# sotelo/parrot

Hardware: AMD Instinct MI355X
Metric: acoustic feature frames/sec (train fwd+bwd+allreduce+clip/Adam) (higher is better)
Workload: dtype f32; 1 GPU; BASELINE configs[1]: 2-layer attention-GRU decoder, h=1024, batch=64 per GPU, T_enc=200, T_dec=800, fp32; cell=gru, layers=2, hidden=1024, batch_per_gpu=64, global_batch=64, T_enc=200, T_dec=800, parallelism=dp1, params=13919212

## Files before the change

### include/parrot_hip.h

```cpp
#ifndef PARROT_HIP_H
#define PARROT_HIP_H

#include <stddef.h>
#include <stdint.h>

#ifdef __cplusplus
extern "C" {
#endif

#define PARROT_ERR_BADARG 10001
#define PARROT_ERR_UNSUPPORTED 10002

#define PARROT_NORM_EPS 1e-5f
#define PARROT_MAX_LAYERS 3

const char* parrot_hip_version(void);

int parrot_profile_begin(void);
long long parrot_profile_end(double* total_us, double* flops, double* bytes);
long long parrot_profile_end2(double* total_us, double* flops, double* bytes, double* plain4);

#define PARROT_PRECISION_F32 0
#define PARROT_PRECISION_BF16 1
#define PARROT_PRECISION_BF16X3 2
int parrot_set_gemm_precision(int mode);
int parrot_get_gemm_precision(void);
int parrot_gemm(const float* A, int lda, int transA, const float* B, int ldb, int transB, float* C, int ldc,
                int M, int N, int K, const float* bias, float alpha, int accumulate, int act, int nbatch,
                long long strideA, long long strideB, long long strideC, int split_k, void* stream);

int parrot_gemm_gated(const float* A, int lda, int transA, const float* B, int ldb, int transB, float* C, int ldc,
                      int M, int N, int K, const float* gate, int ldg, void* stream);

#define PARROT_GEMM_ROUTE_STEP 0
#define PARROT_GEMM_ROUTE_F32 1
#define PARROT_GEMM_ROUTE_BF16 2
#define PARROT_GEMM_ROUTE_BF16X3 3
int parrot_gemm_route(const float* A, int lda, int transA, const float* B, int ldb, int transB, int M, int N, int K,
                      float alpha, int act, int nbatch, long long strideA, long long strideB, int split_k, int has_gate,
                      int* kernel, int* slices);

int parrot_to_bf16(const float* x, void* y, long long n, void* stream);
int parrot_gemm_bf16in(const void* A, int lda, const void* B, int ldb, float* C, int ldc, int M, int N, int K,
                       int accumulate, int split_k, void* stream);
int parrot_gemm_bf16in_ex(const void* A, int lda, int transA, const void* B, int ldb, int transB, float* C, int ldc, int M,
                          int N, int K, const float* bias, int accumulate, int split_k, void* stream);

int parrot_colsum(const float* x, long long M, int N, int ld, float* out, int accumulate, void* stream);

int parrot_gru_step_fwd(const float* h, const float* inputs, const float* gate_inputs, const float* mask,
                        const float* Wg, const float* Wc, float* h_out, float* z, float* r, float* rh,
                        float* c, int B, int H, void* stream);

int parrot_gru_step_bwd(const float* dh_out, const float* h, const float* mask, const float* Wg,
                        const float* Wc, const float* z, const float* r, const float* c, float* dh,
                        float* d_inputs, float* d_gate_inputs, int B, int H, void* stream);

typedef struct ParrotGruSeqDesc {
    int T, B, H, nchain, use_graph, reserved;
    int reverse[4];
    const float* Wg[4];
    const float* Wc[4];
    const float* inputs[4];
    const float* gate_inputs[4];
    const float* mask;
    float* h[4];
    float* z[4]; float* r[4]; float* rh[4]; float* c[4];
    float* dh[4];
    float* dG[4];
    float* dC[4];
} ParrotGruSeqDesc;

int parrot_gru_seq_create(const ParrotGruSeqDesc* desc, void** plan);
int parrot_gru_seq_fwd(void* plan, void* stream);
int parrot_gru_seq_bwd(void* plan, void* stream);
int parrot_gru_seq_destroy(void* plan);

typedef struct ParrotLstmSeqDesc {
    int T, B, H, use_graph;
    const float* W;
    const float* pre_in;
    float* s; float* c;
    float* gates;
    float* dS;
    float* dc;
    float* dP;
} ParrotLstmSeqDesc;

int parrot_lstm_seq_create(const ParrotLstmSeqDesc* desc, void** plan);
int parrot_lstm_seq_fwd(void* plan, void* stream);
int parrot_lstm_seq_bwd(void* plan, void* stream);
int parrot_lstm_seq_destroy(void* plan);

int parrot_gmm_attention_fwd(const float* h1, const float* WattT, const float* batt, const float* kappa_prev,
                             const float* ctx, float* a, float* b, float* kappa, float* phi, float* w, int B,
                             int H, int A, int U, int E, int att_type, float eps, float alignment,
                             float sharpening, float timing, void* stream);

int parrot_gmm_attention_bwd(const float* dw, const float* ctx, const float* a, const float* b,
                             const float* kappa, const float* kappa_prev, const float* WattT, float* dkappa,
                             float* dp, float* dh1, int B, int H, int A, int U, int E, int att_type, float eps,
                             void* stream);

typedef struct ParrotDecoderDesc {
    int T, B, H, E, A, U, L, att_type, use_graph;
    int reserved;
    float eps, alignment, sharpening, timing;
    const float* Wg[PARROT_MAX_LAYERS];
    const float* Wc[PARROT_MAX_LAYERS];
    const float* bg[PARROT_MAX_LAYERS];
    const float* bc[PARROT_MAX_LAYERS];
    const float* WattT;
    const float* batt;
    const float* ctx;
    float* seq_c[PARROT_MAX_LAYERS];
    float* seq_g[PARROT_MAX_LAYERS];
    float* h[PARROT_MAX_LAYERS];
    float* w;
    float* kappa;
    float* z[PARROT_MAX_LAYERS]; float* r[PARROT_MAX_LAYERS];
    float* rh[PARROT_MAX_LAYERS]; float* c[PARROT_MAX_LAYERS];
    float* a; float* b;
    float* phi;
    float* dh[PARROT_MAX_LAYERS];
    float* dw;
    float* dw0;
    float* dhup[PARROT_MAX_LAYERS];
    float* dkappa;
    float* dG[PARROT_MAX_LAYERS];
    float* dC[PARROT_MAX_LAYERS];
    float* dp;
    int cell;
    int seq_init;
    float* cst[PARROT_MAX_LAYERS];
    float* gate4[PARROT_MAX_LAYERS];
    float* dcell[PARROT_MAX_LAYERS];
    int layer_norm, bf16;
    const float* ln_bg[PARROT_MAX_LAYERS * PARROT_MAX_LAYERS];
    const float* ln_bc[PARROT_MAX_LAYERS * PARROT_MAX_LAYERS];
    float* ln_yg[PARROT_MAX_LAYERS * PARROT_MAX_LAYERS];
    float* ln_yc[PARROT_MAX_LAYERS * PARROT_MAX_LAYERS];
    float* ln_sg[PARROT_MAX_LAYERS * PARROT_MAX_LAYERS];
    float* ln_sc[PARROT_MAX_LAYERS * PARROT_MAX_LAYERS];
    const float* Wg_f[PARROT_MAX_LAYERS];
    const float* Wc_f[PARROT_MAX_LAYERS];
    const float* Wg_r[PARROT_MAX_LAYERS];
    const float* Wc_r[PARROT_MAX_LAYERS];
    int* att_sup;
    float* persist_ws;
    long long persist_ws_floats;
    float* dh_b[PARROT_MAX_LAYERS];
    float* dhup_b[PARROT_MAX_LAYERS];
    float* dw_b;
    float* dw0_b;
    float* dhup_c[PARROT_MAX_LAYERS];
    float* dw_c;
    float* dw0_c;
    void* dG16[PARROT_MAX_LAYERS];
} ParrotDecoderDesc;

long long parrot_decoder_persist_floats(const ParrotDecoderDesc* desc);
int parrot_decoder_is_persistent(void* plan);
int parrot_decoder_schedule(void* plan);
int parrot_decoder_backward_tick(void* plan);
long long parrot_decoder_trace(void* plan, int which, long long* out, long long cap);
long long parrot_decoder_trace_jobs(void* plan, int which, long long* out, long long cap);
int parrot_decoder_status(void* plan);

int parrot_decoder_create(const ParrotDecoderDesc* desc, void** plan);
int parrot_decoder_writes_bf16_grads(void* plan);
int parrot_decoder_seq_fwd(void* plan, void* stream);
int parrot_decoder_seq_bwd(void* plan, void* stream);
int parrot_decoder_destroy(void* plan);

#define PARROT_READOUT_MAX_SEG 4
typedef struct ParrotReadoutComposedDesc {
    long long M;
    long long ws_floats;
    int nseg, R, O, zero_rows;
    int slice_rows, nbias;
    int K[PARROT_READOUT_MAX_SEG];
    int ldx[PARROT_READOUT_MAX_SEG];
    int lddx[PARROT_READOUT_MAX_SEG];
    int ldwr, ldwo, ldp, lddp;
    int ldgwr, ldgwo;
    const float* x[PARROT_READOUT_MAX_SEG];
    const float* Wr; const float* Wo;
    const float* rb[PARROT_READOUT_MAX_SEG];
    const float* bo;
    float* pred;
    const float* dp;
    float* dx[PARROT_READOUT_MAX_SEG];
    float* gWr; float* gWo;
    float* grb[PARROT_READOUT_MAX_SEG];
    float* gbo;
} ParrotReadoutComposedDesc;

long long parrot_readout_composed_ws_floats(const ParrotReadoutComposedDesc* desc);
int parrot_readout_composed_fwd(const ParrotReadoutComposedDesc* desc, float* ws, void* stream);
int parrot_readout_composed_bwd(const ParrotReadoutComposedDesc* desc, float* ws, void* stream);

typedef struct ParrotSampleDesc {
    int S, B, H, E, A, U, L, O, R, ldx, att_type, use_graph;
    float eps, alignment, sharpening, timing;
    const float* Wg[PARROT_MAX_LAYERS];
    const float* Wc[PARROT_MAX_LAYERS];
    const float* bg[PARROT_MAX_LAYERS];
    const float* bc[PARROT_MAX_LAYERS];
    const float* Wfg[PARROT_MAX_LAYERS];
    const float* Wfc[PARROT_MAX_LAYERS];
    const float* seq_c[PARROT_MAX_LAYERS];
    const float* seq_g[PARROT_MAX_LAYERS];
    const float* WattT; const float* batt;
    const float* Wr; const float* br;
    const float* radd;
    const float* Wo; const float* bo;
    const float* oadd;
    const float* ctx;
    float* x;
    float* h[PARROT_MAX_LAYERS];
    float* w;
    float* kappa;
    float* a;
    float* bwork;
    float* phi;
    float* zwork; float* rwork; float* rhwork; float* readout;
    int gmm_K, reserved2;
    float sampling_bias, reserved3;
    const float* Wmu; const float* bmu; const float* Wsig; const float* bsig; const float* Wco; const float* bco;
    const float* add_mu; const float* add_sig; const float* add_co;
    const float* unif; const float* noise;
    float* gmm_mu; float* gmm_sig; float* gmm_co;
    float* pi_out;
    int cell, reserved5;
    float* cwork[PARROT_MAX_LAYERS];
    float* gwork;
    int layer_norm, reserved7;
    const float* bfg[PARROT_MAX_LAYERS];
    const float* bfc[PARROT_MAX_LAYERS];
    const float* ln_bg[PARROT_MAX_LAYERS * PARROT_MAX_LAYERS];
    const float* ln_bc[PARROT_MAX_LAYERS * PARROT_MAX_LAYERS];
    const float* br_l[PARROT_MAX_LAYERS];
    float* ln_scratch;
    long long ln_scratch_floats;
    const float* Wg_t[PARROT_MAX_LAYERS];
    const float* Wc_t[PARROT_MAX_LAYERS];
    const float* Wr_t; const float* Wo_t; const float* bo_pad; const float* oadd_pad;
    float* persist_ws;
    long long persist_ws_floats;
    const float* Wro_t;
    const float* ro_const;
    const float* Wgx_t[PARROT_MAX_LAYERS];
    const float* Wcx_t[PARROT_MAX_LAYERS];
    const float* Watt_t;
    int bf16, reserved8;
    const void* Wg_t16[PARROT_MAX_LAYERS];
    const int* eou_pos;
    const int* eou_ncmp;
    int* eou_first;
    int eou_extra, reserved9;
} ParrotSampleDesc;

long long parrot_sample_persist_floats(const ParrotSampleDesc* desc);
int parrot_sample_is_persistent(void* plan);
int parrot_sample_is_bf16(void* plan);
int parrot_sample_plan_pieces_dry(const ParrotSampleDesc* desc, int nwg, int* info16);
int parrot_sample_status(void* plan);
int parrot_sample_stops_early(void* plan);
int parrot_sample_steps_run(void* plan, int* steps);

int parrot_sample_create(const ParrotSampleDesc* desc, void** plan);
int parrot_sample_run(void* plan, void* stream);
int parrot_sample_destroy(void* plan);

int parrot_plan_last_error(void* plan);

int parrot_sumsq(const float* x, size_t n, float* out, void* stream);

int parrot_tile_weights(const float* W, int rows, int cols, int ld, float* out, int mode, int lstm_H, void* stream);
int parrot_tile_weights_bf16(const float* W, int rows, int cols, int ld, void* out, int mode, int lstm_H, void* stream);

int parrot_simple_norm_fwd(const float* x, int ldx, float* y, int ldy, float* sigma, long long R, int N, float eps,
                           float* add_dst, int ld_add, void* stream);
int parrot_simple_norm_bwd(const float* dy, int lddy, const float* y, int ldy, const float* sigma, float* dx,
                           int lddx, long long R, int N, float eps, int accumulate, void* stream);
int parrot_adam_clip_step(float* param, const float* grad, float* m, float* v, size_t n,
                          const float* gnorm_sq, float grad_scale, float clip_threshold, float lr,
                          float beta1, float beta2, float eps, int step, void* stream);

int parrot_batch_quantize(const float* x, int rows, int n, int ld, double* ws, void* out, int ldo, int mode,
                          int q_levels, void* stream);
int parrot_mu2linear(const int32_t* q, size_t n, float* out, void* stream);

int parrot_gather_sum_fwd(const float* tbl, const int* idx, const float* add, int ldadd, float* y, int ldy, long long N,
                          int J, int Q, int D, void* stream);
long long parrot_gather_sum_bwd_ws_floats(long long N, int J, int Q, int D);
int parrot_gather_sum_bwd(const float* dy, int lddy, const int* perm, const int* offs, float* dtbl, float* ws,
                          long long ws_floats, long long N, int J, int Q, int D, int accumulate, void* stream);
int parrot_softmax_ce_fwd(const float* logits, int ld, const int* target, long long rows, int Q, float* lse, float* ce,
                          void* stream);
int parrot_softmax_ce_bwd(const float* logits, int ld, const int* target, const float* lse, const float* rowscale,
                          long long rows, int Q, float* dlogits, int ldd, void* stream);
int parrot_relu_gate(const float* dy, const float* gate, float* out, long long n, void* stream);

int parrot_gmm_cost_fwd(const float* y, int ldy, const float* mu, int ldmu, const float* sig_hat, int ldsig,
                        const float* co_hat, int ldco, long long M, int O, int K, float eps, float* nll, float* pi_out,
                        int ldpi, float* logr, void* stream);
int parrot_gmm_cost_bwd(const float* y, int ldy, const float* mu, int ldmu, const float* sig_hat, int ldsig,
                        const float* co_hat, int ldco, const float* logr, const float* rowscale, long long M, int O, int K,
                        float eps, float* dmu, int lddmu, float* dsig_hat, int lddsig, float* dco_hat, int lddco,
                        void* stream);

long long samplernn_weightnorm_ws_floats(int N);
int samplernn_weightnorm_fold(const float* W, int ld, const float* g, float* W_eff, int ldo, float* norm, float* ws, int K, int N,
                              void* stream);
int samplernn_weightnorm_fold_bwd(const float* W, int ld, const float* g, const float* norm, const float* dW_eff, int ldd,
                                  float* dW, int lddw, float* dg, float* ws, int K, int N, int accumulate_w, int accumulate_g,
                                  void* stream);

typedef struct SampleRnnGenDesc {
    int B, D, T, Q, FS, BFS, feat_dim, use_graph;
    float temperature; int reserved;
    unsigned long long seed;
    const float* big_Win_frames; const float* big_Win_feats; const float* big_bin;
    const float* big_U; const float* big_bU; const float* big_Wg; const float* big_Wc;
    const float* big_Wout; const float* big_bout;
    const float* frm_Win; const float* frm_bin;
    const float* frm_U; const float* frm_bU; const float* frm_Wg; const float* frm_Wc;
    const float* frm_Wout; const float* frm_bout;
    const float* emb_tbl;
    const float* W2; const float* b2; const float* W3; const float* b3; const float* W4; const float* b4;
    const float* features;
    int* samples;
    float* big_h; float* frm_h;
    float* xf_big; float* xf_frm; float* feat_cur; float* gru_in; float* P; float* z; float* r; float* rh;
    float* big_out; float* frame_out; float* o1; float* o2; float* o3; float* logits;
    int* tbase;
    int n_rnn, lstm;
    const float* big_L[5][4];
    const float* frm_L[5][4];
    float* big_hs[5]; float* big_cs[5];
    float* frm_hs[5]; float* frm_cs[5];
    float* gate_ws; float* layer_tmp;
    float* persist_ws;
    long long persist_ws_floats;
} SampleRnnGenDesc;

long long samplernn_persist_floats(const SampleRnnGenDesc* desc);
int samplernn_generate_create(const SampleRnnGenDesc* desc, void** plan);
int samplernn_generate_run(void* plan, void* stream);
int samplernn_generate_is_persistent(void* plan);
int samplernn_generate_status(void* plan);
int samplernn_generate_destroy(void* plan);

#ifdef __cplusplus
}
#endif
#endif
```

### parrot_amd/_lib.py

```python
from __future__ import annotations

import ctypes as C
import os

from .utils import env_str

_HERE = os.path.dirname(os.path.abspath(__file__))
LIB_PATH = os.path.join(_HERE, "libparrot_hip.so")

MAX_LAYERS = 3

c_float_p = C.c_void_p


class HipLibraryMissing(RuntimeError):
    pass


class HipCallError(RuntimeError):
    pass


class GruSeqDesc(C.Structure):
    _fields_ = [
        ("T", C.c_int), ("B", C.c_int), ("H", C.c_int), ("nchain", C.c_int),
        ("use_graph", C.c_int), ("reserved", C.c_int),
        ("reverse", C.c_int * 4),
        ("Wg", C.c_void_p * 4), ("Wc", C.c_void_p * 4),
        ("inputs", C.c_void_p * 4), ("gate_inputs", C.c_void_p * 4),
        ("mask", C.c_void_p),
        ("h", C.c_void_p * 4),
        ("z", C.c_void_p * 4), ("r", C.c_void_p * 4), ("rh", C.c_void_p * 4), ("c", C.c_void_p * 4),
        ("dh", C.c_void_p * 4), ("dG", C.c_void_p * 4), ("dC", C.c_void_p * 4),
    ]


class LstmSeqDesc(C.Structure):
    _fields_ = [(n, C.c_int) for n in ("T", "B", "H", "use_graph")] + \
               [(n, C.c_void_p) for n in ("W", "pre_in", "s", "c", "gates", "dS", "dc", "dP")]


class DecoderDesc(C.Structure):
    _fields_ = [
        ("T", C.c_int), ("B", C.c_int), ("H", C.c_int), ("E", C.c_int), ("A", C.c_int),
        ("U", C.c_int), ("L", C.c_int), ("att_type", C.c_int), ("use_graph", C.c_int),
        ("reserved", C.c_int),
        ("eps", C.c_float), ("alignment", C.c_float), ("sharpening", C.c_float), ("timing", C.c_float),
        ("Wg", C.c_void_p * MAX_LAYERS), ("Wc", C.c_void_p * MAX_LAYERS),
        ("bg", C.c_void_p * MAX_LAYERS), ("bc", C.c_void_p * MAX_LAYERS),
        ("WattT", C.c_void_p), ("batt", C.c_void_p), ("ctx", C.c_void_p),
        ("seq_c", C.c_void_p * MAX_LAYERS), ("seq_g", C.c_void_p * MAX_LAYERS),
        ("h", C.c_void_p * MAX_LAYERS), ("w", C.c_void_p), ("kappa", C.c_void_p),
        ("z", C.c_void_p * MAX_LAYERS), ("r", C.c_void_p * MAX_LAYERS),
        ("rh", C.c_void_p * MAX_LAYERS), ("c", C.c_void_p * MAX_LAYERS),
        ("a", C.c_void_p), ("b", C.c_void_p), ("phi", C.c_void_p),
        ("dh", C.c_void_p * MAX_LAYERS), ("dw", C.c_void_p), ("dw0", C.c_void_p), ("dhup", C.c_void_p * MAX_LAYERS),
        ("dkappa", C.c_void_p),
        ("dG", C.c_void_p * MAX_LAYERS), ("dC", C.c_void_p * MAX_LAYERS), ("dp", C.c_void_p),
        ("cell", C.c_int), ("seq_init", C.c_int),
        ("cst", C.c_void_p * MAX_LAYERS), ("gate4", C.c_void_p * MAX_LAYERS), ("dcell", C.c_void_p * MAX_LAYERS),
        ("layer_norm", C.c_int), ("bf16", C.c_int),
        ("ln_bg", C.c_void_p * (MAX_LAYERS * MAX_LAYERS)), ("ln_bc", C.c_void_p * (MAX_LAYERS * MAX_LAYERS)),
        ("ln_yg", C.c_void_p * (MAX_LAYERS * MAX_LAYERS)), ("ln_yc", C.c_void_p * (MAX_LAYERS * MAX_LAYERS)),
        ("ln_sg", C.c_void_p * (MAX_LAYERS * MAX_LAYERS)), ("ln_sc", C.c_void_p * (MAX_LAYERS * MAX_LAYERS)),
        ("Wg_f", C.c_void_p * MAX_LAYERS), ("Wc_f", C.c_void_p * MAX_LAYERS),
        ("Wg_r", C.c_void_p * MAX_LAYERS), ("Wc_r", C.c_void_p * MAX_LAYERS),
        ("att_sup", C.c_void_p),
        ("persist_ws", C.c_void_p), ("persist_ws_floats", C.c_longlong),
        ("dh_b", C.c_void_p * MAX_LAYERS), ("dhup_b", C.c_void_p * MAX_LAYERS), ("dw_b", C.c_void_p), ("dw0_b", C.c_void_p),
        ("dhup_c", C.c_void_p * MAX_LAYERS), ("dw_c", C.c_void_p), ("dw0_c", C.c_void_p),
        ("dG16", C.c_void_p * MAX_LAYERS),
    ]


READOUT_MAX_SEG = 4


class ReadoutComposedDesc(C.Structure):
    _fields_ = [
        ("M", C.c_longlong), ("ws_floats", C.c_longlong),
        ("nseg", C.c_int), ("R", C.c_int), ("O", C.c_int), ("zero_rows", C.c_int),
        ("slice_rows", C.c_int), ("nbias", C.c_int),
        ("K", C.c_int * READOUT_MAX_SEG), ("ldx", C.c_int * READOUT_MAX_SEG), ("lddx", C.c_int * READOUT_MAX_SEG),
        ("ldwr", C.c_int), ("ldwo", C.c_int), ("ldp", C.c_int), ("lddp", C.c_int),
        ("ldgwr", C.c_int), ("ldgwo", C.c_int),
        ("x", C.c_void_p * READOUT_MAX_SEG),
        ("Wr", C.c_void_p), ("Wo", C.c_void_p),
        ("rb", C.c_void_p * READOUT_MAX_SEG), ("bo", C.c_void_p),
        ("pred", C.c_void_p), ("dp", C.c_void_p),
        ("dx", C.c_void_p * READOUT_MAX_SEG),
        ("gWr", C.c_void_p), ("gWo", C.c_void_p),
        ("grb", C.c_void_p * READOUT_MAX_SEG), ("gbo", C.c_void_p),
    ]


class SampleDesc(C.Structure):
    _fields_ = [
        ("S", C.c_int), ("B", C.c_int), ("H", C.c_int), ("E", C.c_int), ("A", C.c_int),
        ("U", C.c_int), ("L", C.c_int), ("O", C.c_int), ("R", C.c_int), ("ldx", C.c_int),
        ("att_type", C.c_int), ("use_graph", C.c_int),
        ("eps", C.c_float), ("alignment", C.c_float), ("sharpening", C.c_float), ("timing", C.c_float),
        ("Wg", C.c_void_p * MAX_LAYERS), ("Wc", C.c_void_p * MAX_LAYERS),
        ("bg", C.c_void_p * MAX_LAYERS), ("bc", C.c_void_p * MAX_LAYERS),
        ("Wfg", C.c_void_p * MAX_LAYERS), ("Wfc", C.c_void_p * MAX_LAYERS),
        ("seq_c", C.c_void_p * MAX_LAYERS), ("seq_g", C.c_void_p * MAX_LAYERS),
        ("WattT", C.c_void_p), ("batt", C.c_void_p),
        ("Wr", C.c_void_p), ("br", C.c_void_p), ("radd", C.c_void_p),
        ("Wo", C.c_void_p), ("bo", C.c_void_p), ("oadd", C.c_void_p),
        ("ctx", C.c_void_p),
        ("x", C.c_void_p), ("h", C.c_void_p * MAX_LAYERS), ("w", C.c_void_p), ("kappa", C.c_void_p),
        ("a", C.c_void_p), ("bwork", C.c_void_p), ("phi", C.c_void_p),
        ("zwork", C.c_void_p), ("rwork", C.c_void_p), ("rhwork", C.c_void_p), ("readout", C.c_void_p),
        ("gmm_K", C.c_int), ("reserved2", C.c_int), ("sampling_bias", C.c_float), ("reserved3", C.c_float),
        ("Wmu", C.c_void_p), ("bmu", C.c_void_p), ("Wsig", C.c_void_p), ("bsig", C.c_void_p),
        ("Wco", C.c_void_p), ("bco", C.c_void_p),
        ("add_mu", C.c_void_p), ("add_sig", C.c_void_p), ("add_co", C.c_void_p),
        ("unif", C.c_void_p), ("noise", C.c_void_p),
        ("gmm_mu", C.c_void_p), ("gmm_sig", C.c_void_p), ("gmm_co", C.c_void_p), ("pi_out", C.c_void_p),
        ("cell", C.c_int), ("reserved5", C.c_int),
        ("cwork", C.c_void_p * MAX_LAYERS), ("gwork", C.c_void_p),
        ("layer_norm", C.c_int), ("reserved7", C.c_int),
        ("bfg", C.c_void_p * MAX_LAYERS), ("bfc", C.c_void_p * MAX_LAYERS),
        ("ln_bg", C.c_void_p * (MAX_LAYERS * MAX_LAYERS)), ("ln_bc", C.c_void_p * (MAX_LAYERS * MAX_LAYERS)),
        ("br_l", C.c_void_p * MAX_LAYERS),
        ("ln_scratch", C.c_void_p), ("ln_scratch_floats", C.c_longlong),
        ("Wg_t", C.c_void_p * MAX_LAYERS), ("Wc_t", C.c_void_p * MAX_LAYERS),
        ("Wr_t", C.c_void_p), ("Wo_t", C.c_void_p), ("bo_pad", C.c_void_p), ("oadd_pad", C.c_void_p),
        ("persist_ws", C.c_void_p), ("persist_ws_floats", C.c_longlong),
        ("Wro_t", C.c_void_p), ("ro_const", C.c_void_p),
        ("Wgx_t", C.c_void_p * MAX_LAYERS), ("Wcx_t", C.c_void_p * MAX_LAYERS),
        ("Watt_t", C.c_void_p),
        ("bf16", C.c_int), ("reserved8", C.c_int),
        ("Wg_t16", C.c_void_p * MAX_LAYERS),
        ("eou_pos", C.c_void_p), ("eou_ncmp", C.c_void_p), ("eou_first", C.c_void_p),
        ("eou_extra", C.c_int), ("reserved9", C.c_int),
    ]


class SampleRnnGenDesc(C.Structure):
    _fields_ = ([(n, C.c_int) for n in ("B", "D", "T", "Q", "FS", "BFS", "feat_dim", "use_graph")] +
                [("temperature", C.c_float), ("reserved", C.c_int), ("seed", C.c_ulonglong)] +
                [(n, C.c_void_p) for n in (
                    "big_Win_frames", "big_Win_feats", "big_bin", "big_U", "big_bU", "big_Wg", "big_Wc",
                    "big_Wout", "big_bout", "frm_Win", "frm_bin", "frm_U", "frm_bU", "frm_Wg", "frm_Wc",
                    "frm_Wout", "frm_bout", "emb_tbl", "W2", "b2", "W3", "b3", "W4", "b4", "features",
                    "samples", "big_h", "frm_h", "xf_big", "xf_frm", "feat_cur", "gru_in", "P", "z", "r", "rh",
                    "big_out", "frame_out", "o1", "o2", "o3", "logits", "tbase")] +
                [("n_rnn", C.c_int), ("lstm", C.c_int),
                 ("big_L", (C.c_void_p * 4) * 5), ("frm_L", (C.c_void_p * 4) * 5),
                 ("big_hs", C.c_void_p * 5), ("big_cs", C.c_void_p * 5),
                 ("frm_hs", C.c_void_p * 5), ("frm_cs", C.c_void_p * 5),
                 ("gate_ws", C.c_void_p), ("layer_tmp", C.c_void_p),
                 ("persist_ws", C.c_void_p), ("persist_ws_floats", C.c_longlong)])


_vp, _i, _f, _ll, _sz = C.c_void_p, C.c_int, C.c_float, C.c_longlong, C.c_size_t
SIGNATURES = {
    "parrot_hip_version": (C.c_char_p, []),
    "parrot_profile_begin": (_i, []),
    "parrot_profile_end": (C.c_longlong, [C.POINTER(C.c_double)] * 3),
    "parrot_profile_end2": (C.c_longlong, [C.POINTER(C.c_double)] * 4),
    "parrot_gemm": (_i, [_vp, _i, _i, _vp, _i, _i, _vp, _i, _i, _i, _i, _vp, _f, _i, _i, _i, _ll, _ll, _ll, _i, _vp]),
    "parrot_gemm_gated": (_i, [_vp, _i, _i, _vp, _i, _i, _vp, _i, _i, _i, _i, _vp, _i, _vp]),
    "parrot_gemm_route": (_i, [_vp, _i, _i, _vp, _i, _i, _i, _i, _i, _f, _i, _i, _ll, _ll, _i, _i,
                               C.POINTER(C.c_int), C.POINTER(C.c_int)]),
    "parrot_gather_sum_fwd": (_i, [_vp, _vp, _vp, _i, _vp, _i, _ll, _i, _i, _i, _vp]),
    "parrot_gather_sum_bwd_ws_floats": (C.c_longlong, [_ll, _i, _i, _i]),
    "parrot_gather_sum_bwd": (_i, [_vp, _i, _vp, _vp, _vp, _vp, _ll, _ll, _i, _i, _i, _i, _vp]),
    "parrot_softmax_ce_fwd": (_i, [_vp, _i, _vp, _ll, _i, _vp, _vp, _vp]),
    "parrot_softmax_ce_bwd": (_i, [_vp, _i, _vp, _vp, _vp, _ll, _i, _vp, _i, _vp]),
    "parrot_relu_gate": (_i, [_vp, _vp, _vp, _ll, _vp]),
    "parrot_gmm_cost_fwd": (_i, [_vp, _i] * 4 + [_ll, _i, _i, _f, _vp, _vp, _i, _vp, _vp]),
    "parrot_gmm_cost_bwd": (_i, [_vp, _i] * 4 + [_vp, _vp, _ll, _i, _i, _f] + [_vp, _i] * 3 + [_vp]),
    "samplernn_weightnorm_ws_floats": (_ll, [_i]),
    "samplernn_weightnorm_fold": (_i, [_vp, _i, _vp, _vp, _i, _vp, _vp, _i, _i, _vp]),
    "samplernn_weightnorm_fold_bwd": (_i, [_vp, _i, _vp, _vp, _vp, _i, _vp, _i, _vp, _vp, _i, _i, _i, _i, _vp]),
    "parrot_colsum": (_i, [_vp, _ll, _i, _i, _vp, _i, _vp]),
    "parrot_gru_step_fwd": (_i, [_vp] * 11 + [_i, _i, _vp]),
    "parrot_gru_step_bwd": (_i, [_vp] * 11 + [_i, _i, _vp]),
    "parrot_gru_seq_create": (_i, [C.POINTER(GruSeqDesc), C.POINTER(C.c_void_p)]),
    "parrot_gru_seq_fwd": (_i, [_vp, _vp]),
    "parrot_gru_seq_bwd": (_i, [_vp, _vp]),
    "parrot_gru_seq_destroy": (_i, [_vp]),
    "parrot_lstm_seq_create": (_i, [C.POINTER(LstmSeqDesc), C.POINTER(C.c_void_p)]),
    "parrot_lstm_seq_fwd": (_i, [_vp, _vp]),
    "parrot_lstm_seq_bwd": (_i, [_vp, _vp]),
    "parrot_lstm_seq_destroy": (_i, [_vp]),
    "parrot_gmm_attention_fwd": (_i, [_vp] * 10 + [_i] * 6 + [_f] * 4 + [_vp]),
    "parrot_gmm_attention_bwd": (_i, [_vp] * 10 + [_i] * 6 + [_f, _vp]),
    "parrot_decoder_create": (_i, [C.POINTER(DecoderDesc), C.POINTER(C.c_void_p)]),
    "parrot_decoder_persist_floats": (C.c_longlong, [C.POINTER(DecoderDesc)]),
    "parrot_decoder_is_persistent": (_i, [_vp]),
    "parrot_decoder_schedule": (_i, [_vp]),
    "parrot_decoder_backward_tick": (_i, [_vp]),
    "parrot_decoder_writes_bf16_grads": (_i, [_vp]),
    "parrot_decoder_trace": (C.c_longlong, [_vp, _i, C.POINTER(C.c_longlong), C.c_longlong]),
    "parrot_decoder_trace_jobs": (C.c_longlong, [_vp, _i, C.POINTER(C.c_longlong), C.c_longlong]),
    "parrot_decoder_seq_fwd": (_i, [_vp, _vp]),
    "parrot_decoder_seq_bwd": (_i, [_vp, _vp]),
    "parrot_decoder_destroy": (_i, [_vp]),
    "parrot_readout_composed_ws_floats": (C.c_longlong, [C.POINTER(ReadoutComposedDesc)]),
    "parrot_readout_composed_fwd": (_i, [C.POINTER(ReadoutComposedDesc), _vp, _vp]),
    "parrot_readout_composed_bwd": (_i, [C.POINTER(ReadoutComposedDesc), _vp, _vp]),
    "parrot_sample_create": (_i, [C.POINTER(SampleDesc), C.POINTER(C.c_void_p)]),
    "parrot_sample_persist_floats": (C.c_longlong, [C.POINTER(SampleDesc)]),
    "parrot_sample_is_persistent": (_i, [_vp]),
    "parrot_sample_is_bf16": (_i, [_vp]),
    "parrot_sample_plan_pieces_dry": (_i, [C.POINTER(SampleDesc), _i, C.POINTER(C.c_int)]),
    "parrot_sample_status": (_i, [_vp]),
    "parrot_sample_stops_early": (_i, [_vp]),
    "parrot_sample_steps_run": (_i, [_vp, C.POINTER(C.c_int)]),
    "parrot_decoder_status": (_i, [_vp]),
    "parrot_sample_run": (_i, [_vp, _vp]),
    "parrot_sample_destroy": (_i, [_vp]),
    "parrot_plan_last_error": (_i, [_vp]),
    "parrot_sumsq": (_i, [_vp, _sz, _vp, _vp]),
    "parrot_tile_weights": (_i, [_vp, _i, _i, _i, _vp, _i, _i, _vp]),
    "parrot_tile_weights_bf16": (_i, [_vp, _i, _i, _i, _vp, _i, _i, _vp]),
    "parrot_set_gemm_precision": (_i, [_i]),
    "parrot_get_gemm_precision": (_i, []),
    "parrot_to_bf16": (_i, [_vp, _vp, _ll, _vp]),
    "parrot_gemm_bf16in": (_i, [_vp, _i, _vp, _i, _vp, _i, _i, _i, _i, _i, _i, _vp]),
    "parrot_gemm_bf16in_ex": (_i, [_vp, _i, _i, _vp, _i, _i, _vp, _i, _i, _i, _i, _vp, _i, _i, _vp]),
    "parrot_simple_norm_fwd": (_i, [_vp, _i, _vp, _i, _vp, _ll, _i, _f, _vp, _i, _vp]),
    "parrot_simple_norm_bwd": (_i, [_vp, _i, _vp, _i, _vp, _vp, _i, _ll, _i, _f, _i, _vp]),
    "parrot_adam_clip_step": (_i, [_vp, _vp, _vp, _vp, _sz, _vp, _f, _f, _f, _f, _f, _f, _i, _vp]),
    "parrot_batch_quantize": (_i, [_vp, _i, _i, _i, _vp, _vp, _i, _i, _i, _vp]),
    "parrot_mu2linear": (_i, [_vp, _sz, _vp, _vp]),
    "samplernn_generate_create": (_i, [C.POINTER(SampleRnnGenDesc), C.POINTER(C.c_void_p)]),
    "samplernn_generate_run": (_i, [_vp, _vp]),
    "samplernn_persist_floats": (C.c_longlong, [C.POINTER(SampleRnnGenDesc)]),
    "samplernn_generate_is_persistent": (_i, [_vp]),
    "samplernn_generate_status": (_i, [_vp]),
    "samplernn_generate_destroy": (_i, [_vp]),
}

_lib = None


def load():
    global _lib
    if _lib is not None:
        return _lib
    import torch
    path = env_str('PARROT_HIP_LIB', LIB_PATH)
    if not os.path.exists(path):
        raise HipLibraryMissing(
            f"{LIB_PATH} not found: build it with `python -m parrot_amd.build` "
            "(hipcc --offload-arch=gfx950).  There is no CPU fallback for the product path.")
    lib = C.CDLL(path)
    for name, (res, args) in SIGNATURES.items():
        fn = getattr(lib, name)
        fn.restype = res
        fn.argtypes = args
    _lib = lib
    return lib


def check(rc: int, what: str, plan=None):
    if rc != 0:
        raise HipCallError(f"{what} failed with code {rc}")


def call(name: str, *args):
    lib = load()
    rc = getattr(lib, name)(*args)
    check(rc, name)
    return rc
```

### parrot_amd/build.py

```python
from __future__ import annotations

import hashlib
import os
import subprocess
import sys
from concurrent.futures import ThreadPoolExecutor

from .utils import env_str

HERE = os.path.dirname(os.path.abspath(__file__))
CSRC = os.path.join(HERE, "csrc")
OUT = os.path.join(HERE, "libparrot_hip.so")
OBJDIR = os.path.join(CSRC, "build")
ARCH = "gfx950"

SOURCES = ["skinny.hip", "biggemm.hip", "attention.hip", "elementwise.hip", "quantize.hip",
           "plans.hip", "plans_decode.hip", "capi.hip", "samplernn.hip", "persist.hip", "sr_persist.hip", "rowgru.hip", "trainops.hip", "readout.hip",
           "gmmcost.hip"]
EXTRA_FLAGS = {"quantize.hip": ["-ffp-contract=off"]}
if env_str("PARROT_PM_DEPTH"):
    EXTRA_FLAGS["persist.hip"] = ["-DPM_DEPTH=" + env_str("PARROT_PM_DEPTH")]


def _hipcc() -> str:
    for cand in (os.environ.get("HIPCC"), "/opt/rocm/bin/hipcc", "hipcc"):
        if cand and (os.path.isabs(cand) and os.path.exists(cand) or not os.path.isabs(cand)):
            return cand
    return "hipcc"


def _digest(paths) -> str:
    h = hashlib.sha256()
    for p in sorted(paths):
        with open(p, "rb") as f:
            h.update(p.encode())
            h.update(f.read())
    return h.hexdigest()


def build(force: bool = False, verbose: bool = True, timers: bool = False) -> str:
    global OUT, OBJDIR
    if timers:
        OUT = os.path.join(HERE, "libparrot_hip_timers.so")
        OBJDIR = os.path.join(CSRC, "build_timers")
    tag, extra = env_str("PARROT_BUILD_TAG"), env_str("PARROT_BUILD_FLAGS", "").split()
    if tag:
        OUT = os.path.join(HERE, f"libparrot_hip_{tag}.so")
        OBJDIR = os.path.join(CSRC, f"build_{tag}")
    srcs = [s for s in SOURCES if os.path.exists(os.path.join(CSRC, s))]
    deps = [os.path.join(CSRC, f) for f in os.listdir(CSRC) if f.endswith((".hip", ".h"))]
    deps.append(os.path.join(HERE, "..", "include", "parrot_hip.h"))
    stamp = os.path.join(OBJDIR, "stamp.txt")
    dig = _digest(deps)
    if not force and os.path.exists(OUT) and os.path.exists(stamp) and open(stamp).read() == dig:
        return OUT
    os.makedirs(OBJDIR, exist_ok=True)
    hipcc = _hipcc()
    common = [hipcc, f"--offload-arch={ARCH}", "-O3", "-std=c++17", "-fPIC"] + (["-DSK_TIMERS"] if timers else []) + (extra if tag else [])

    def compile_one(src):
        obj = os.path.join(OBJDIR, src.replace(".hip", ".o"))
        cmd = common + EXTRA_FLAGS.get(src, []) + ["-c", os.path.join(CSRC, src), "-o", obj]
        r = subprocess.run(cmd, capture_output=True, text=True)
        if r.returncode != 0:
            raise RuntimeError(f"hipcc failed for {src}:\n{r.stdout}\n{r.stderr}")
        return obj

    with ThreadPoolExecutor(max_workers=min(8, len(srcs))) as ex:
        objs = list(ex.map(compile_one, srcs))
    cmd = [hipcc, f"--offload-arch={ARCH}", "-shared", "-fPIC", "-o", OUT] + objs
    r = subprocess.run(cmd, capture_output=True, text=True)
    if r.returncode != 0:
        raise RuntimeError(f"link failed:\n{r.stdout}\n{r.stderr}")
    with open(stamp, "w") as f:
        f.write(dig)
    if verbose:
        print(f"[parrot_amd.build] built {OUT}")
    return OUT


if __name__ == "__main__":
    build(force="--force" in sys.argv, timers="--timers" in sys.argv)
```

### parrot_amd/csrc/plans.hip

```cpp
#include "pm_builder.h"
#include "switches.h"

namespace {

struct GruSeqPlan : PlanBase {
    ParrotGruSeqDesc d;

    bool rowwise = false;
    float* tiled = nullptr;
    ~GruSeqPlan() override {
        if (tiled) (void)hipFree(tiled);
    }
    int setup_rowwise() {
        rowwise = rowgru_supported(d.T, d.B, d.H, d.nchain) && env_int("PARROT_GRU_ROWWISE", 1) != 0;
        for (int ch = 0; ch < d.nchain && rowwise; ++ch)
            if (!d.Wg[ch] || !d.Wc[ch] || ((uintptr_t)d.Wg[ch] & 15) || ((uintptr_t)d.Wc[ch] & 15)) rowwise = false;
        if (!rowwise) return 0;
        const size_t per = (size_t)6 * d.H * d.H;
        if (hipMalloc(&tiled, sizeof(float) * per * d.nchain) != hipSuccess) {
            tiled = nullptr;
            rowwise = false;
        }
        return 0;
    }
    RowGruArgs row_args() const {
        RowGruArgs g;
        memset(&g, 0, sizeof(g));
        const size_t HH = (size_t)d.H * d.H;
        for (int ch = 0; ch < d.nchain; ++ch) {
            RowGruChain& c = g.chain[ch];
            float* base = tiled + (size_t)ch * 6 * HH;
            c.Wg_f = base; c.Wc_f = base + 2 * HH; c.Wg_r = base + 3 * HH; c.Wc_r = base + 5 * HH;
            c.inputs = d.inputs[ch]; c.gate_inputs = d.gate_inputs[ch];
            c.h = d.h[ch]; c.z = d.z[ch]; c.r = d.r[ch]; c.rh = d.rh[ch]; c.c = d.c[ch];
            c.dh = d.dh[ch]; c.dG = d.dG[ch]; c.dC = d.dC[ch];
            c.reverse = d.reverse[ch];
        }
        g.mask = d.mask; g.T = d.T; g.B = d.B; g.H = d.H; g.nchain = d.nchain;
        return g;
    }
    int fwd_rowwise(hipStream_t st) {
        const RowGruArgs g = row_args();
        for (int ch = 0; ch < d.nchain; ++ch) {
            const RowGruChain& c = g.chain[ch];
            PL_TRY(sk_tile_weights_launch(d.Wg[ch], d.H, 2 * d.H, 2 * d.H, const_cast<float*>(c.Wg_f), 0, 0, st));
            PL_TRY(sk_tile_weights_launch(d.Wc[ch], d.H, d.H, d.H, const_cast<float*>(c.Wc_f), 0, 0, st));
            PL_TRY(sk_tile_weights_launch(d.Wg[ch], d.H, 2 * d.H, 2 * d.H, const_cast<float*>(c.Wg_r), 1, 0, st));
            PL_TRY(sk_tile_weights_launch(d.Wc[ch], d.H, d.H, d.H, const_cast<float*>(c.Wc_r), 1, 0, st));
        }
        return rowgru_fwd_launch(g, st);
    }

    int enqueue(int which, hipStream_t s) override {
        if (rowwise) return which == 0 ? fwd_rowwise(s) : rowgru_bwd_launch(row_args(), s);
        return which == 0 ? fwd(s) : bwd(s);
    }

    int fwd(hipStream_t st) {
        const size_t BH = (size_t)d.B * d.H;
        for (int s = 0; s < d.T; ++s) {
            SkJob jobs[4];
            for (int ch = 0; ch < d.nchain; ++ch) {
                const int t = d.reverse[ch] ? d.T - 1 - s : s;
                SkJob& j = jobs[ch];
                sk_job_init(j);
                j.nseg = 1;
                j.seg[0] = sk_seg(d.h[ch] + s * BH, d.H, d.Wg[ch], 2 * d.H, d.H, 0);
                j.M = d.B; j.N = 2 * d.H; j.H = d.H; j.epi = SK_EPI_GRU_GATES;
                j.add = d.gate_inputs[ch] ? d.gate_inputs[ch] + t * 2 * BH : nullptr; j.ld_add = 2 * d.H;
                j.e0 = d.h[ch] + s * BH; j.lde0 = d.H;
                j.o1 = d.z[ch] + t * BH; j.ldo1 = d.H;
                j.o2 = d.r[ch] + t * BH; j.ldo2 = d.H;
                j.out = d.rh[ch] + t * BH; j.ldo = d.H;
            }
            PL_TRY(launch_jobs(jobs, d.nchain, st));
            for (int ch = 0; ch < d.nchain; ++ch) {
                const int t = d.reverse[ch] ? d.T - 1 - s : s;
                SkJob& j = jobs[ch];
                sk_job_init(j);
                j.nseg = 1;
                j.seg[0] = sk_seg(d.rh[ch] + t * BH, d.H, d.Wc[ch], d.H, d.H, 0);
                j.M = d.B; j.N = d.H; j.H = d.H; j.epi = SK_EPI_GRU_CAND;
                j.add = d.inputs[ch] ? d.inputs[ch] + t * BH : nullptr; j.ld_add = d.H;
                j.e0 = d.h[ch] + s * BH; j.lde0 = d.H;
                j.e1 = d.z[ch] + t * BH; j.lde1 = d.H;
                j.o1 = d.c[ch] + t * BH; j.ldo1 = d.H;
                j.out = d.h[ch] + (s + 1) * BH; j.ldo = d.H;
                j.mask = d.mask ? d.mask + (size_t)t * d.B : nullptr;
            }
            PL_TRY(launch_jobs(jobs, d.nchain, st));
        }
        return 0;
    }

    int bwd(hipStream_t st) {
        const size_t BH = (size_t)d.B * d.H;
        for (int s = d.T - 1; s >= 0; --s) {
            GruStateBwdArgs ga;
            ga.nchain = d.nchain; ga.B = d.B; ga.H = d.H;
            SkJob jx[4], jy[4];
            for (int ch = 0; ch < d.nchain; ++ch) {
                const int t = d.reverse[ch] ? d.T - 1 - s : s;
                GruStateBwdChain& c = ga.chain[ch];
                c.dh = d.dh[ch] + (s + 1) * BH;
                c.dh2 = nullptr;
                c.hprev = d.h[ch] + s * BH;
                c.z = d.z[ch] + t * BH;
                c.c = d.c[ch] + t * BH;
                c.mask = d.mask ? d.mask + (size_t)t * d.B : nullptr;
                c.dC = d.dC[ch] + t * BH;
                c.dG = d.dG[ch] + t * 2 * BH;
                c.dhprev = d.dh[ch] + s * BH;

                SkJob& x = jx[ch];
                sk_job_init(x);
                x.nseg = 1;
                x.seg[0] = sk_seg(d.dC[ch] + t * BH, d.H, d.Wc[ch], d.H, d.H, 1);
                x.M = d.B; x.N = d.H; x.H = d.H; x.epi = SK_EPI_BWD_RH;
                x.e0 = d.h[ch] + s * BH; x.lde0 = d.H;
                x.e1 = d.r[ch] + t * BH; x.lde1 = d.H;
                x.out = d.dG[ch] + t * 2 * BH + d.H; x.ldo = 2 * d.H;
                x.o1 = d.dh[ch] + s * BH; x.ldo1 = d.H;

                SkJob& y = jy[ch];
                sk_job_init(y);
                y.nseg = 1;
                y.seg[0] = sk_seg(d.dG[ch] + t * 2 * BH, 2 * d.H, d.Wg[ch], 2 * d.H, 2 * d.H, 1);
                y.M = d.B; y.N = d.H; y.H = d.H; y.epi = SK_EPI_LINEAR; y.accumulate = 1;
                y.out = d.dh[ch] + s * BH; y.ldo = d.H;
            }
            PL_TRY(gru_state_bwd_launch(ga, st));
            PL_TRY(launch_jobs(jx, d.nchain, st));
            PL_TRY(launch_jobs(jy, d.nchain, st));
        }
        return 0;
    }
};

struct LstmSeqPlan : PlanBase {
    ParrotLstmSeqDesc d;
    int enqueue(int which, hipStream_t s) override { return which == 0 ? fwd(s) : bwd(s); }

    int fwd(hipStream_t st) {
        const size_t BH = (size_t)d.B * d.H;
        for (int t = 0; t < d.T; ++t) {
            SkJob j;
            sk_job_init(j);
            j.nseg = 1;
            j.seg[0] = sk_seg(d.s + t * BH, d.H, d.W, 4 * d.H, d.H, 0);
            j.M = d.B; j.N = 4 * d.H; j.H = d.H; j.epi = SK_EPI_LSTM;
            j.add = d.pre_in + (size_t)t * 4 * BH; j.ld_add = 4 * d.H;
            j.e1 = d.c + t * BH; j.lde1 = d.H;
            j.o1 = d.c + (t + 1) * BH; j.ldo1 = d.H;
            j.o2 = d.gates + (size_t)t * 4 * BH; j.ldo2 = 4 * d.H;
            j.out = d.s + (t + 1) * BH; j.ldo = d.H;
            PL_TRY(launch_jobs(&j, 1, st));
        }
        return 0;
    }

    int bwd(hipStream_t st) {
        const size_t BH = (size_t)d.B * d.H;
        for (int t = d.T - 1; t >= 0; --t) {
            PL_TRY(lstm_state_bwd_launch(d.dS + (t + 1) * BH, nullptr, d.dc, d.gates + (size_t)t * 4 * BH, d.c + t * BH,
                                         d.c + (t + 1) * BH, d.dP + (size_t)t * 4 * BH, d.B, d.H, st));
            SkJob y;
            sk_job_init(y);
            y.nseg = 1;
            y.seg[0] = sk_seg(d.dP + (size_t)t * 4 * BH, 4 * d.H, d.W, 4 * d.H, 4 * d.H, 1);
            y.M = d.B; y.N = d.H; y.H = d.H; y.epi = SK_EPI_LINEAR; y.accumulate = 1;
            y.out = d.dS + t * BH; y.ldo = d.H;
            PL_TRY(launch_jobs(&y, 1, st));
        }
        return 0;
    }
};

struct DecoderPlan : PlanBase {
    ParrotDecoderDesc d;

    int schedule = 0, chunk = 50;
    int esplit = 1;
    int full_wgs = 0;
    bool tiled = false;
    bool s5_w_in_step = true;
    unsigned* att_flags = nullptr;
    unsigned* bwd_flags = nullptr;
    bool flags_fake = false;
    bool bwd_fused = false;
    bool bwd_ksplit = false;
    bool bwd_hetero = false;
    bool persist_ok = false;
    PmProgram pm_prog;

    ~DecoderPlan() override {
        if (att_flags && !flags_fake) (void)hipFree(att_flags);
        if (bwd_flags && !flags_fake) (void)hipFree(bwd_flags);
    }

    int run(int which, hipStream_t s) override {
        BgPrecisionScope precision(d.bf16 ? 1 : -1);
        return PlanBase::run(which, s);
    }

    int enqueue(int which, hipStream_t s) override {
        BgPrecisionScope precision(d.bf16 ? 1 : -1);
        if (which == 0 && persist_ok) return pm_launch(pm_prog, s);
        if (schedule == 3) return which == 0 ? fwd_skew(s) : bwd_skew(s);
        if (which == 1 && bwd_hetero && (schedule == 0 || schedule == 5)) return bwd8(s);
        if (schedule == 5) return which == 0 ? fwd5(s) : bwd(s);
        if (schedule == 7) return which == 0 ? fwd7(s) : bwd(s);
        return which == 0 ? fwd(s) : bwd(s);
    }

    int trace(int which, std::vector<TraceRec>& out, std::vector<TraceJob>* jobs_out = nullptr) {
        if (persist_ok || (schedule != 0 && schedule < 5) || d.layer_norm) return PARROT_ERR_UNSUPPORTED;
        Tracer tr;
        g_tracer = &tr;
        const int rc = enqueue(which, nullptr);
        g_tracer = nullptr;
        out.swap(tr.recs);
        if (jobs_out) jobs_out->swap(tr.jobs);
        return rc;
    }

    int krows(int l) const { return d.H + d.E + l * d.H; }
    float* dctx(float* of_l0, float* of_upper, int l, int t) const {
        const size_t BE = (size_t)d.B * d.E;
        return l == 0 ? of_l0 + (size_t)t * BE : of_upper + (size_t)(t + 1) * BE;
    }
    SkSeg fseg(const float* A, int lda, int l, int g, int r0, int K, int ldw) const {
        if (tiled) {
            const float* Wt = g == 0 ? d.Wg_f[l] : d.Wc_f[l];
            if (d.bf16) return sk_seg(A, lda, Wt + (size_t)(r0 >> 5) * 256, (krows(l) >> 5) * 256, K, 3);
            return sk_seg(A, lda, Wt + (size_t)(r0 >> 4) * 256, (krows(l) >> 4) * 256, K, 2);
        }
        const float* W = g == 0 ? d.Wg[l] : d.Wc[l];
        return sk_seg(A, lda, W + (size_t)r0 * ldw, ldw, K, 0);
    }
    SkSeg rseg(const float* A, int l, int g, int r0, int ldw) const {
        if (tiled) {
            const float* Wt = g == 0 ? d.Wg_r[l] : d.Wc_r[l];
            if (d.bf16) return sk_seg(A, ldw, Wt + (size_t)(r0 >> 4) * (ldw >> 5) * 256, (ldw >> 5) * 256, ldw, 3);
            return sk_seg(A, ldw, Wt + (size_t)(r0 >> 4) * (ldw >> 4) * 256, (ldw >> 4) * 256, ldw, 2);
        }
        const float* W = g == 0 ? d.Wg[l] : d.Wc[l];
        return sk_seg(A, ldw, W + (size_t)r0 * ldw, ldw, ldw, 1);
    }
    SkSeg rseg_k(const float* A, int l, int g, int r0, int ldw, int k0, int K) const {
        const float* Wt = g == 0 ? d.Wg_r[l] : d.Wc_r[l];
        return sk_seg(A + k0, ldw, Wt + ((size_t)(r0 >> 4) * (ldw >> 4) + (k0 >> 4)) * 256, (ldw >> 4) * 256, K, 2);
    }

    void layer_segs(SkJob& j, int l, int t, const float* first, int g, int ldw) const {
        const size_t BH = (size_t)d.B * d.H, BE = (size_t)d.B * d.E;
        int n = 0;
        j.seg[n++] = fseg(first, d.H, l, g, 0, d.H, ldw);
        const float* wsrc = d.w + (size_t)(l == 0 ? t : t + 1) * BE;
        j.seg[n++] = fseg(wsrc, d.E, l, g, d.H, d.E, ldw);
        for (int q = 0; q < l; ++q)
            j.seg[n++] = fseg(d.h[q] + (size_t)(t + 1) * BH, d.H, l, g, d.H + d.E + q * d.H, d.H, ldw);
        j.nseg = n;
    }
    void own_segs(SkJob& j, int l, int t, const float* first, int g, int ldw) const {
        const size_t BE = (size_t)d.B * d.E;
        j.seg[0] = fseg(first, d.H, l, g, 0, d.H, ldw);
        j.nseg = 1;
        if (l == 0) j.seg[j.nseg++] = fseg(d.w + (size_t)t * BE, d.E, l, g, d.H, d.E, ldw);
    }

    bool has_seq(int l, const float* p) const { return p && (((d.seq_init >> l) & 1) || (schedule >= 2 && schedule != 7 && l > 0)); }

    void gates_job(SkJob& j, int l, int t) const {
        const size_t BH = (size_t)d.B * d.H;
        sk_job_init(j);
        layer_segs(j, l, t, d.h[l] + t * BH, 0, 2 * d.H);
        j.M = d.B; j.N = 2 * d.H; j.H = d.H; j.epi = SK_EPI_GRU_GATES;
        j.bias = d.bg[l];
        j.add = has_seq(l, d.seq_g[l]) ? d.seq_g[l] + t * 2 * BH : nullptr; j.ld_add = 2 * d.H;
        j.e0 = d.h[l] + t * BH; j.lde0 = d.H;
        j.o1 = d.z[l] + t * BH; j.ldo1 = d.H;
        j.o2 = d.r[l] + t * BH; j.ldo2 = d.H;
        j.out = d.rh[l] + t * BH; j.ldo = d.H;
    }

    void cand_job(SkJob& j, int l, int t) const {
        const size_t BH = (size_t)d.B * d.H;
        sk_job_init(j);
        layer_segs(j, l, t, d.rh[l] + t * BH, 1, d.H);
        j.M = d.B; j.N = d.H; j.H = d.H; j.epi = SK_EPI_GRU_CAND;
        j.bias = d.bc[l];
        j.add = has_seq(l, d.seq_c[l]) ? d.seq_c[l] + t * BH : nullptr; j.ld_add = d.H;
        j.e0 = d.h[l] + t * BH; j.lde0 = d.H;
        j.e1 = d.z[l] + t * BH; j.lde1 = d.H;
        j.o1 = d.c[l] + t * BH; j.ldo1 = d.H;
        j.out = d.h[l] + (t + 1) * BH; j.ldo = d.H;
    }

    void lstm_job(SkJob& j, int l, int t) const {
        const size_t BH = (size_t)d.B * d.H;
        sk_job_init(j);
        layer_segs(j, l, t, d.h[l] + t * BH, 0, 4 * d.H);
        j.M = d.B; j.N = 4 * d.H; j.H = d.H; j.epi = SK_EPI_LSTM;
        j.bias = d.bg[l];
        j.add = has_seq(l, d.seq_g[l]) ? d.seq_g[l] + t * 4 * BH : nullptr; j.ld_add = 4 * d.H;
        j.e1 = d.cst[l] + t * BH; j.lde1 = d.H;
        j.o1 = d.cst[l] + (t + 1) * BH; j.ldo1 = d.H;
        j.o2 = d.gate4[l] + t * 4 * BH; j.ldo2 = 4 * d.H;
        j.out = d.h[l] + (t + 1) * BH; j.ldo = d.H;
    }

    void input_job(SkJob& j, int l, int t, int g, int part = 0, bool no_w = false) const {
        const size_t BH = (size_t)d.B * d.H, BE = (size_t)d.B * d.E;
        const int wd = d.cell == 1 ? 4 * d.H : (g == 0 ? 2 * d.H : d.H);
        sk_job_init(j);
        j.colmode = d.cell == 1 && tiled ? 1 : 0;
        int n = 0;
        if (part != 2 && !no_w) j.seg[n++] = fseg(d.w + (size_t)(t + 1) * BE, d.E, l, g, d.H, d.E, wd);
        for (int q = 0; q < l; ++q) {
            if ((part == 1 && q == l - 1) || (part == 2 && q != l - 1)) continue;
            j.seg[n++] = fseg(d.h[q] + (size_t)(t + 1) * BH, d.H, l, g, d.H + d.E + q * d.H, d.H, wd);
        }
        j.nseg = n;
        j.M = d.B; j.N = wd; j.H = d.H; j.epi = SK_EPI_LINEAR;
        float* sq = (g == 0 ? d.seq_g[l] : d.seq_c[l]) + (size_t)t * d.B * wd;
        j.out = sq; j.ldo = wd;
        j.accumulate = part == 2 ? 1 : ((d.seq_init >> l) & 1);
    }

    AttFwdArgs att_fwd_args(int t) const {
        const size_t BH = (size_t)d.B * d.H, BE = (size_t)d.B * d.E, BA = (size_t)d.B * d.A;
        AttFwdArgs g{};
        g.h1 = d.h[0] + (t + 1) * BH; g.ldh = d.H;
        g.WattT = d.WattT; g.batt = d.batt;
        g.kappa_prev = d.kappa + t * BA;
        g.ctx = d.ctx;
        g.a_out = d.a + t * BA; g.b_out = d.b + t * BA; g.kappa_out = d.kappa + (t + 1) * BA;
        g.phi_out = d.phi + (size_t)t * d.B * d.U;
        g.w_out = d.w + (t + 1) * BE; g.ldw = d.E;
        g.B = d.B; g.H = d.H; g.A = d.A; g.U = d.U; g.E = d.E; g.esplit = esplit;
        g.att_type = d.att_type; g.eps = d.eps; g.alignment = d.alignment;
// ... 868 lines not shown
```

### parrot_amd/csrc/rowgru.h

```cpp
#pragma once
#include "common.h"

struct RowGruChain {
    const float* Wg_f; const float* Wc_f;
    const float* Wg_r; const float* Wc_r;
    const float* inputs;
    const float* gate_inputs;
    float* h;
    float* z; float* r; float* rh; float* c;
    float* dh;
    float* dG; float* dC;
    int reverse, pad;
};

struct RowGruArgs {
    RowGruChain chain[4];
    const float* mask;
    int T, B, H, nchain;
};

bool rowgru_supported(int T, int B, int H, int nchain);
int rowgru_fwd_launch(const RowGruArgs& g, hipStream_t stream);
int rowgru_bwd_launch(const RowGruArgs& g, hipStream_t stream);
```

### parrot_amd/csrc/rowgru.hip

```cpp
#include "rowgru.h"

#include "skinny.h"

namespace {

constexpr int RG_THREADS = 256, RG_ROWS = 16, RG_MAXH = 128;

__device__ __forceinline__ float rg_sigmoid(float x) { return 1.0f / (1.0f + expf(-x)); }

template <int NT, int NCH>
__device__ __forceinline__ void rg_load_w(const float* __restrict__ Bt, int ct0, int ntiles, int lane, f32x4 (&wb)[NT][NCH]) {
#pragma unroll
    for (int q = 0; q < NT; ++q) {
        const int ct = min(ct0 + 4 * q, ntiles - 1);
#pragma unroll
        for (int c = 0; c < NCH; ++c) wb[q][c] = *reinterpret_cast<const f32x4*>(Bt + ((size_t)ct * NCH + c) * 256 + 4 * lane);
    }
}
template <int NT, int NCH>
__device__ __forceinline__ void rg_mma(const float* __restrict__ A, int lda, const f32x4 (&wb)[NT][NCH], int lane, f32x4 (&acc)[NT]) {
    const int kk = lane >> 4, i = lane & 15;
#pragma unroll
    for (int q = 0; q < NT; ++q) acc[q] = (f32x4){0.f, 0.f, 0.f, 0.f};
#pragma unroll
    for (int c = 0; c < NCH; ++c) {
        const f32x4 a = *reinterpret_cast<const f32x4*>(A + i * lda + 16 * c + 4 * kk);
#pragma unroll
        for (int u = 0; u < 4; ++u)
#pragma unroll
            for (int q = 0; q < NT; ++q) acc[q] = __builtin_amdgcn_mfma_f32_16x16x4f32(a[u], wb[q][c][u], acc[q], 0, 0, 0);
    }
}

template <int NCH>
__global__ __launch_bounds__(RG_THREADS) void rg_fwd_kernel(const RowGruArgs g) {
    constexpr int NTG = (2 * NCH + 3) / 4, NTC = (NCH + 3) / 4;
    extern __shared__ __attribute__((aligned(16))) float sm[];
    const int H = g.H, B = g.B, T = g.T, P = H + 4;
    float* s_h = sm;
    float* s_rh = s_h + RG_ROWS * P;
    float* s_z = s_rh + RG_ROWS * P;
    const int ch = blockIdx.y, m0 = blockIdx.x * RG_ROWS;
    const int tid = threadIdx.x, lane = tid & 63, wave = tid >> 6;
    const RowGruChain& c = g.chain[ch];
    const size_t BH = (size_t)B * H;
    const int ntg = (2 * H) >> 4, ntc = H >> 4;
    f32x4 wg[NTG][NCH], wc[NTC][NCH];
    rg_load_w<NTG, NCH>(c.Wg_f, wave, ntg, lane, wg);
    rg_load_w<NTC, NCH>(c.Wc_f, wave, ntc, lane, wc);
    for (int e = tid; e < RG_ROWS * H; e += RG_THREADS) {
        const int m = e / H, k = e % H;
        s_h[m * P + k] = (m0 + m < B) ? c.h[(size_t)(m0 + m) * H + k] : 0.f;
    }
    __syncthreads();
    const int gq = lane >> 4, jj = lane & 15;
    float pg[NTG][4], pc[NTC][4];
    auto prefetch = [&](int s) {
        const int t = c.reverse ? T - 1 - s : s;
#pragma unroll
        for (int q = 0; q < NTG; ++q)
#pragma unroll
            for (int r = 0; r < 4; ++r) {
                const int n = 16 * (wave + 4 * q) + jj, mr = m0 + 4 * gq + r;
                pg[q][r] = (c.gate_inputs && s < T && wave + 4 * q < ntg && mr < B)
                               ? c.gate_inputs[(size_t)t * 2 * BH + (size_t)mr * 2 * H + n] : 0.f;
            }
#pragma unroll
        for (int q = 0; q < NTC; ++q)
#pragma unroll
            for (int r = 0; r < 4; ++r) {
                const int n = 16 * (wave + 4 * q) + jj, mr = m0 + 4 * gq + r;
                pc[q][r] = (c.inputs && s < T && wave + 4 * q < ntc && mr < B) ? c.inputs[(size_t)t * BH + (size_t)mr * H + n] : 0.f;
            }
    };
    prefetch(0);
    for (int s = 0; s < T; ++s) {
        const int t = c.reverse ? T - 1 - s : s;
        float cg[NTG][4], cc_in[NTC][4];
#pragma unroll
        for (int q = 0; q < NTG; ++q)
#pragma unroll
            for (int r = 0; r < 4; ++r) cg[q][r] = pg[q][r];
#pragma unroll
        for (int q = 0; q < NTC; ++q)
#pragma unroll
            for (int r = 0; r < 4; ++r) cc_in[q][r] = pc[q][r];
        prefetch(s + 1);
        {
            f32x4 acc[NTG];
            rg_mma<NTG, NCH>(s_h, P, wg, lane, acc);
#pragma unroll
            for (int q = 0; q < NTG; ++q) {
                const int ct = wave + 4 * q;
                if (ct >= ntg) continue;
                const int n = 16 * ct + jj;
#pragma unroll
                for (int r = 0; r < 4; ++r) {
                    const int m = 4 * gq + r, mr = m0 + m;
                    if (mr >= B) continue;
                    const float pre = acc[q][r] + cg[q][r];
                    const float gt = rg_sigmoid(pre);
                    if (n < H) {
                        c.z[(size_t)t * BH + (size_t)mr * H + n] = gt;
                        s_z[m * P + n] = gt;
                    } else {
                        const int j = n - H;
                        c.r[(size_t)t * BH + (size_t)mr * H + j] = gt;
                        const float rh = gt * s_h[m * P + j];
                        c.rh[(size_t)t * BH + (size_t)mr * H + j] = rh;
                        s_rh[m * P + j] = rh;
                    }
                }
            }
        }
        __syncthreads();
        {
            f32x4 acc[NTC];
            rg_mma<NTC, NCH>(s_rh, P, wc, lane, acc);
#pragma unroll
            for (int q = 0; q < NTC; ++q) {
                const int ct = wave + 4 * q;
                if (ct >= ntc) continue;
                const int n = 16 * ct + jj;
#pragma unroll
                for (int r = 0; r < 4; ++r) {
                    const int m = 4 * gq + r, mr = m0 + m;
                    if (mr >= B) continue;
                    const float pre = acc[q][r] + cc_in[q][r];
                    const float cc = tanhf(pre);
                    const float z = s_z[m * P + n], hp = s_h[m * P + n];
                    float hn = z * cc + (1.f - z) * hp;
                    if (g.mask) {
                        const float mk = g.mask[(size_t)t * B + mr];
                        hn = mk * hn + (1.f - mk) * hp;
                    }
                    c.c[(size_t)t * BH + (size_t)mr * H + n] = cc;
                    c.h[(size_t)(s + 1) * BH + (size_t)mr * H + n] = hn;
                    s_h[m * P + n] = hn;
                }
            }
        }
        __syncthreads();
    }
}

template <int NCH>
__global__ __launch_bounds__(RG_THREADS) void rg_bwd_kernel(const RowGruArgs g) {
    constexpr int NTC = (NCH + 3) / 4;
    extern __shared__ __attribute__((aligned(16))) float sm[];
    const int H = g.H, B = g.B, T = g.T, P = H + 4, P2 = 2 * H + 4;
    float* s_cur = sm;
    float* s_dC = s_cur + RG_ROWS * P;
    float* s_dhp = s_dC + RG_ROWS * P;
    float* s_dG = s_dhp + RG_ROWS * P;
    const int ch = blockIdx.y, m0 = blockIdx.x * RG_ROWS;
    const int tid = threadIdx.x, lane = tid & 63, wave = tid >> 6;
    const RowGruChain& c = g.chain[ch];
    const size_t BH = (size_t)B * H;
    const int ntc = H >> 4;
    f32x4 wx[NTC][NCH], wy[NTC][2 * NCH];
    rg_load_w<NTC, NCH>(c.Wc_r, wave, ntc, lane, wx);
    rg_load_w<NTC, 2 * NCH>(c.Wg_r, wave, ntc, lane, wy);
    for (int e = tid; e < RG_ROWS * H; e += RG_THREADS) {
        const int m = e / H, k = e % H;
        s_cur[m * P + k] = (m0 + m < B) ? c.dh[(size_t)T * BH + (size_t)(m0 + m) * H + k] : 0.f;
    }
    __syncthreads();
    const int gq = lane >> 4, jj = lane & 15;
    float p_hp[NCH], p_z[NCH], p_c[NCH], p_r[NTC][4], p_hp2[NTC][4], p_slot[NTC][4];
    auto prefetch = [&](int s) {
        const int t = c.reverse ? T - 1 - s : s;
#pragma unroll
        for (int i = 0; i < NCH; ++i) {
            const int e = tid + RG_THREADS * i, m = e / H, k = e % H, mr = m0 + m;
            const bool ok = s >= 0 && mr < B;
            const size_t ix = ok ? (size_t)t * BH + (size_t)mr * H + k : 0;
            p_hp[i] = ok ? c.h[(size_t)s * BH + (size_t)mr * H + k] : 0.f;
            p_z[i] = ok ? c.z[ix] : 0.f;
            p_c[i] = ok ? c.c[ix] : 0.f;
        }
#pragma unroll
        for (int q = 0; q < NTC; ++q)
#pragma unroll
            for (int r = 0; r < 4; ++r) {
                const int n = 16 * (wave + 4 * q) + jj, mr = m0 + 4 * gq + r;
                const bool ok = s >= 0 && wave + 4 * q < ntc && mr < B;
                p_r[q][r] = ok ? c.r[(size_t)t * BH + (size_t)mr * H + n] : 0.f;
                p_hp2[q][r] = ok ? c.h[(size_t)s * BH + (size_t)mr * H + n] : 0.f;
                p_slot[q][r] = ok ? c.dh[(size_t)s * BH + (size_t)mr * H + n] : 0.f;
            }
    };
    prefetch(T - 1);
    for (int s = T - 1; s >= 0; --s) {
        const int t = c.reverse ? T - 1 - s : s;
        float q_hp[NCH], q_z[NCH], q_c[NCH], q_r[NTC][4], q_hp2[NTC][4], q_slot[NTC][4];
#pragma unroll
        for (int i = 0; i < NCH; ++i) { q_hp[i] = p_hp[i]; q_z[i] = p_z[i]; q_c[i] = p_c[i]; }
#pragma unroll
        for (int q = 0; q < NTC; ++q)
#pragma unroll
            for (int r = 0; r < 4; ++r) { q_r[q][r] = p_r[q][r]; q_hp2[q][r] = p_hp2[q][r]; q_slot[q][r] = p_slot[q][r]; }
        prefetch(s - 1);
#pragma unroll
        for (int ei = 0; ei < NCH; ++ei) {
            const int e = tid + RG_THREADS * ei;
            const int m = e / H, k = e % H, mr = m0 + m;
            float dC = 0.f, dGz = 0.f, dhp = 0.f;
            if (mr < B) {
                const size_t i = (size_t)t * BH + (size_t)mr * H + k;
                float dh = s_cur[m * P + k];
                const float hp = q_hp[ei];
                float direct = 0.f;
                if (g.mask) {
                    const float mk = g.mask[(size_t)t * B + mr];
                    direct = dh * (1.f - mk);
                    dh *= mk;
                }
                const float z = q_z[ei], cc = q_c[ei];
                dC = dh * z * (1.f - cc * cc);
                dGz = dh * (cc - hp) * z * (1.f - z);
                dhp = dh * (1.f - z) + direct;
                c.dC[i] = dC;
                c.dG[(size_t)t * 2 * BH + (size_t)mr * 2 * H + k] = dGz;
            }
            s_dC[m * P + k] = dC;
            s_dG[m * P2 + k] = dGz;
            s_dhp[m * P + k] = dhp;
        }
        __syncthreads();
        {
            f32x4 acc[NTC];
            rg_mma<NTC, NCH>(s_dC, P, wx, lane, acc);
#pragma unroll
            for (int q = 0; q < NTC; ++q) {
                const int ct = wave + 4 * q;
                if (ct >= ntc) continue;
                const int n = 16 * ct + jj;
#pragma unroll
                for (int r = 0; r < 4; ++r) {
                    const int m = 4 * gq + r, mr = m0 + m;
                    float dGr = 0.f;
                    if (mr < B) {
                        const float x = acc[q][r];
                        const float r_ = q_r[q][r];
                        const float hp = q_hp2[q][r];
                        dGr = x * hp * r_ * (1.f - r_);
                        c.dG[(size_t)t * 2 * BH + (size_t)mr * 2 * H + H + n] = dGr;
                        s_dhp[m * P + n] += x * r_;
                    }
                    s_dG[m * P2 + H + n] = dGr;
                }
            }
        }
        __syncthreads();
        {
            f32x4 acc[NTC];
            rg_mma<NTC, 2 * NCH>(s_dG, P2, wy, lane, acc);
#pragma unroll
            for (int q = 0; q < NTC; ++q) {
                const int ct = wave + 4 * q;
                if (ct >= ntc) continue;
                const int n = 16 * ct + jj;
#pragma unroll
                for (int r = 0; r < 4; ++r) {
                    const int m = 4 * gq + r, mr = m0 + m;
                    if (mr >= B) continue;
                    float* slot = c.dh + (size_t)s * BH + (size_t)mr * H + n;
                    const float tot = q_slot[q][r] + (s_dhp[m * P + n] + acc[q][r]);
                    *slot = tot;
                    s_cur[m * P + n] = tot;
                }
            }
        }
        __syncthreads();
    }
}

}

bool rowgru_supported(int T, int B, int H, int nchain) {
    return T >= 1 && B >= 1 && H >= 16 && H <= RG_MAXH && (H % 16) == 0 && nchain >= 1 && nchain <= 4;
}

template <int NCH>
static void rg_launch(int which, const RowGruArgs& g, dim3 grid, size_t lds, hipStream_t stream) {
    if (which == 0) hipLaunchKernelGGL((rg_fwd_kernel<NCH>), grid, dim3(RG_THREADS), lds, stream, g);
    else hipLaunchKernelGGL((rg_bwd_kernel<NCH>), grid, dim3(RG_THREADS), lds, stream, g);
}
static int rg_dispatch(int which, const RowGruArgs& g, hipStream_t stream) {
    if (!rowgru_supported(g.T, g.B, g.H, g.nchain)) return PH_ERR_UNSUPPORTED;
    const dim3 grid(ceil_div(g.B, RG_ROWS), g.nchain);
    const size_t lds = which == 0 ? sizeof(float) * 3 * RG_ROWS * (g.H + 4)
                                  : sizeof(float) * RG_ROWS * (3 * (g.H + 4) + 2 * g.H + 4);
    switch (g.H >> 4) {
        case 1: rg_launch<1>(which, g, grid, lds, stream); break;
        case 2: rg_launch<2>(which, g, grid, lds, stream); break;
        case 3: rg_launch<3>(which, g, grid, lds, stream); break;
        case 4: rg_launch<4>(which, g, grid, lds, stream); break;
        case 5: rg_launch<5>(which, g, grid, lds, stream); break;
        case 6: rg_launch<6>(which, g, grid, lds, stream); break;
        case 7: rg_launch<7>(which, g, grid, lds, stream); break;
        default: rg_launch<8>(which, g, grid, lds, stream); break;
    }
    return (int)hipGetLastError();
}

int rowgru_fwd_launch(const RowGruArgs& g, hipStream_t stream) { return rg_dispatch(0, g, stream); }
int rowgru_bwd_launch(const RowGruArgs& g, hipStream_t stream) { return rg_dispatch(1, g, stream); }
```

### parrot_amd/csrc/switches.h

```cpp
#pragma once
#include <stdlib.h>

static inline int env_int(const char* name, int dflt) {
    const char* e = getenv(name);
    return e ? atoi(e) : dflt;
}
static inline bool env_set(const char* name) { return getenv(name) != nullptr; }
static inline const char* env_str(const char* name) { return getenv(name); }

static inline int sw_att_dense() { return env_int("PARROT_ATT_DENSE", 0); }
static inline int sw_pm_dataflow(int dflt) { return env_int("PARROT_PM_DATAFLOW", dflt); }
static inline int sw_wk() { return env_int("PARROT_WK", 1); }
static inline bool sw_pm_dump_plan() { return env_set("PARROT_PM_DUMP_PLAN"); }
```

### parrot_amd/model.py

```python
from __future__ import annotations

import collections
import ctypes as C
from collections import OrderedDict

import numpy
import torch

from . import _lib, ops
from .bricks import Brick, Constant, IsotropicGaussian
from .params import ParamStore
from .utils import env_int

floatX = "float32"


def _simple_norm(x, eps=1e-5):
    return (x - x.mean(-1, keepdim=True)) / (eps + x.std(-1, unbiased=False, keepdim=True))


def logsumexp(x, axis=None):
    x_max = x.max(axis, keepdim=True)[0]
    z = torch.log(torch.exp(x - x_max).sum(axis, keepdim=True)) + x_max
    return z.sum(axis)
# ... 45 lines not shown

    def clear(self):
        while len(self):
            _, old = self.popitem(last=False)
            self.on_evict(old)


class Parrot(Brick):
    def __init__(
            self,
            input_dim=420, output_dim=63, rnn_h_dim=1024, readouts_dim=1024,
            weak_feedback=False, full_feedback=False, feedback_noise_level=None,
            layer_norm=False, use_speaker=False, num_speakers=21, speaker_dim=128,
            which_cost='MSE', k_gmm=20, sampling_bias=0, epsilon=1e-5, num_characters=43,
            attention_type='graves', attention_size=10, attention_alignment=1.,
            sharpening_coeff=1., timing_coeff=1., encoder_type=None, encoder_dim=128,
            raw_output=False,
            num_layers=3, encoder_literal=True, use_graph=True, seed=1234,
            cell_type='gru', lstm_forget_bias=3.0, compute_dtype='float32', decode_dtype='float32',
            **kwargs):
        kwargs.setdefault('name', 'parrot')
        kwargs.setdefault('weights_init', IsotropicGaussian(0.01))
        kwargs.setdefault('biases_init', Constant(0.))
        super().__init__(seed=seed, **kwargs)
        assert which_cost in ('MSE', 'GMM')
        assert attention_type in ('graves', 'softmax')
        assert encoder_type in (None, 'bidirectional')
        assert 1 <= num_layers <= _lib.MAX_LAYERS
        assert cell_type in ('gru', 'lstm')
        assert compute_dtype in ('float32', 'bf16', 'bfloat16')
        self.compute_bf16 = compute_dtype != 'float32'
        assert decode_dtype in ('float32', 'bf16', 'bfloat16')
        self.decode_bf16 = decode_dtype != 'float32'
        self.input_dim, self.output_dim = input_dim, output_dim
        self.rnn_h_dim, self.readouts_dim = rnn_h_dim, readouts_dim
        self.layer_norm, self.which_cost, self.use_speaker = layer_norm, which_cost, use_speaker
        self.full_feedback = full_feedback
        self.weak_feedback = bool(weak_feedback or full_feedback)
        self.feedback_noise_level = feedback_noise_level
        self.epsilon = epsilon
        self.num_characters, self.attention_type = num_characters, attention_type
        self.attention_alignment, self.attention_size = attention_alignment, attention_size
        self.sharpening_coeff, self.timing_coeff = sharpening_coeff, timing_coeff
        self.encoder_type, self.encoder_dim = encoder_type, encoder_dim
        self.encoded_input_dim = 2 * encoder_dim if encoder_type == 'bidirectional' else input_dim
        self.raw_output = raw_output
        self.num_speakers, self.speaker_dim = num_speakers, speaker_dim
        self.k_gmm, self.sampling_bias = k_gmm, sampling_bias
        self.num_layers, self.encoder_literal, self.use_graph = num_layers, encoder_literal, use_graph
        self.cell_type, self.lstm_forget_bias = cell_type, float(lstm_forget_bias)
        H_ = rnn_h_dim
        if cell_type == 'lstm':
            self._groups = [('g', 4 * H_, 'inputs', 'dec.Wg', 'W_state')]
        else:
            self._groups = [('g', 2 * H_, 'gates', 'dec.Wg', 'state_to_gates'),
                            ('c', H_, 'inputs', 'dec.Wc', 'state_to_state')]

        self.store = ParamStore()
        self._declare_parameters()
        self._allocated = False
        cap = max(4, env_int('PARROT_WS_CACHE', 6))
        self._train_ws = _LRU(cap, self._evict_train_ws)
        self._sample_ws = _LRU(max(2, cap // 2), self._evict_sample_ws)
        self._carry = {}
        self._token = 0
        self._saved = None
        if raw_output:
            from .sampleRNN.models.conditional import three_tier
            self.sampleRnn = SampleRnn(name='samplernn', device=self.device)

    def _declare_parameters(self):
        s = self.store
        H, R, O, E = self.rnn_h_dim, self.readouts_dim, self.output_dim, self.encoded_input_dim
        A, L = self.attention_size, self.num_layers
        P = '/' + self.name

        def fork_separate(name, din, outs):
            for on, od in outs:
                s.add(f'{P}/{name}/fork_{on}.W', (din, od), 'weight')
                s.add(f'{P}/{name}/fork_{on}.b', (od,), 'bias')

        if self.encoder_type == 'bidirectional':
            D, ED = self.input_dim, self.encoder_dim
            s.add(f'{P}/encoder/embed_label.W', (self.num_characters, D), 'weight')
            for d in ('forward', 'backward'):
                q = f'{P}/encoder/encoder/{d}'
                s.add(f'{q}/fork/fork_inputs.W', (D, ED), 'weight')
                s.add(f'{q}/fork/fork_inputs.b', (ED,), 'bias')
                s.add(f'{q}/fork/fork_gate_inputs.W', (D, 2 * ED), 'weight')
                s.add(f'{q}/fork/fork_gate_inputs.b', (2 * ED,), 'bias')
                s.add(f'{q}/gatedrecurrent.state_to_state', (ED, ED), 'weight')
                s.add(f'{q}/gatedrecurrent.state_to_gates', (ED, 2 * ED), 'weight')
                s.add(f'{q}/gatedrecurrent.initial_state', (ED,), 'initial_state')
        for l in range(1, L + 1):
            K = H + E + (l - 1) * H
            for key, wd, suf, mat, rec in self._groups:
                s.add(f'{mat}{l}', (K, wd), 'weight', alias=False)
            for key, wd, suf, mat, rec in reversed(self._groups):
                s.alias(f'{P}/rnn{l}.{rec}', f'{mat}{l}', rows=(0, H))
            s.add(f'{P}/rnn{l}.initial_state', (H,), 'initial_state')
            if self.cell_type == 'lstm':
                s.add(f'{P}/rnn{l}.initial_cells', (H,), 'initial_state')
            for key, wd, suf, mat, rec in reversed(self._groups):
                s.alias(f'{P}/inp_to_h{l}/fork_rnn{l}_{suf}.W', f'{mat}{l}', rows=(H, H + E))
                s.add(f'{P}/inp_to_h{l}/fork_rnn{l}_{suf}.b', (wd,), 'bias')
            for j in range(1, l):
                r0 = H + E + (j - 1) * H
                for key, wd, suf, mat, rec in reversed(self._groups):
                    s.alias(f'{P}/h{j}_to_h{l}/fork_rnn{l}_{suf}.W', f'{mat}{l}', rows=(r0, r0 + H))
                    s.add(f'{P}/h{j}_to_h{l}/fork_rnn{l}_{suf}.b', (wd,), 'bias')
        s.add('dec.WattT', (3 * A, H), 'weight', alias=False)
        s.add('dec.batt', (3 * A,), 'bias', alias=False)
        for i, n in enumerate(('alpha', 'beta', 'kappa')):
            s.alias(f'{P}/h1_to_att/fork_{n}.W', 'dec.WattT', rows=(i * A, (i + 1) * A), transpose=True)
            s.alias(f'{P}/h1_to_att/fork_{n}.b', 'dec.batt', rows=(i * A, (i + 1) * A), role='bias')
        s.add('dec.Wr', (L * H + E, R), 'weight', alias=False)
        for l in range(1, L + 1):
            s.alias(f'{P}/h{l}_to_readout.W', 'dec.Wr', rows=((l - 1) * H, l * H))
            s.add(f'{P}/h{l}_to_readout.b', (R,), 'bias')
        s.alias(f'{P}/att_to_readout.W', 'dec.Wr', rows=(L * H, L * H + E))
        s.add(f'{P}/att_to_readout.b', (R,), 'bias')
        if self.which_cost == 'MSE':
            s.add(f'{P}/readout_to_output.W', (R, O), 'weight')
            s.add(f'{P}/readout_to_output.b', (O,), 'bias')
            self._out_names = [(f'{P}/readout_to_output.W', f'{P}/readout_to_output.b', O)]
        else:
            K = self.k_gmm
            fork_separate('readout_to_output', R, [('gmm_mu', O * K), ('gmm_sigma', O * K), ('gmm_coeff', K)])
            self._out_names = [(f'{P}/readout_to_output/fork_{n}.W', f'{P}/readout_to_output/fork_{n}.b', d)
                               for n, d in (('gmm_mu', O * K), ('gmm_sigma', O * K), ('gmm_coeff', K))]
        if self.use_speaker:
            SD = self.speaker_dim
            s.add(f'{P}/lookuptable.W', (self.num_speakers, SD), 'weight')
            for l in range(1, L + 1):
                fork_separate(f'speaker_to_h{l}', SD, self._fork_outs(l))
            s.add(f'{P}/speaker_to_readout.W', (SD, R), 'weight')
            s.add(f'{P}/speaker_to_readout.b', (R,), 'bias')
            if self.which_cost == 'MSE':
                s.add(f'{P}/speaker_to_output.W', (SD, O), 'weight')
                s.add(f'{P}/speaker_to_output.b', (O,), 'bias')
                self._spk_out_names = [(f'{P}/speaker_to_output.W', f'{P}/speaker_to_output.b', O)]
            else:
                K = self.k_gmm
                fork_separate('speaker_to_output', SD,
                              [('gmm_mu', O * K), ('gmm_sigma', O * K), ('gmm_coeff', K)])
                self._spk_out_names = [
                    (f'{P}/speaker_to_output/fork_{n}.W', f'{P}/speaker_to_output/fork_{n}.b', d)
                    for n, d in (('gmm_mu', O * K), ('gmm_sigma', O * K), ('gmm_coeff', K))]
        self._fb_layers = []
        if self.weak_feedback:
            self._fb_layers = [1]
        if self.full_feedback:
            self._fb_layers = list(range(1, L + 1))
        for l in self._fb_layers:
            fork_separate(f'out_to_h{l}', O, self._fork_outs(l))
        s.add(f'{P}.initial_w', (E,), 'initial_state')

    def _fork_outs(self, l):
        return [(f'rnn{l}_{suf}', wd) for key, wd, suf, mat, rec in reversed(self._groups)]

    def allocate(self):
        if not self._allocated:
            self.store.allocate(self._dev())
            self._allocated = True
        return self

    def initialize(self, gen=None):
        self.allocate()
        if gen is None:
            gen = torch.Generator().manual_seed(int(self.seed))
        with torch.no_grad():
            for name in self.store.names():
                t = self.store.param(name)
                role = self.store.role(name)
                if role == 'weight':
                    t.copy_(self.weights_init.generate(gen, tuple(t.shape)).to(t.device))
                elif role == 'bias':
                    t.copy_(self.biases_init.generate(gen, tuple(t.shape)).to(t.device))
                else:
                    t.zero_()
            if self.cell_type == 'lstm':
                H = self.rnn_h_dim
                for l in range(1, self.num_layers + 1):
                    self._p(f'/inp_to_h{l}/fork_rnn{l}_inputs.b')[H:2 * H].add_(self.lstm_forget_bias)
        self.initialized = True
        return self

    def get_parameter_dict(self, prefix=""):
        self.allocate()
        return self.store.named_parameters()

    def get_parameter_values(self):
        return OrderedDict((k, v.detach().cpu().numpy().copy()) for k, v in self.get_parameter_dict().items())

    def set_parameter_values(self, values):
        self.allocate()
        with torch.no_grad():
            for k, v in values.items():
                if k not in self.store._aliases:
                    raise KeyError(f'unknown parameter {k}')
                t = self.store.param(k)
                v = torch.as_tensor(numpy.asarray(v) if not isinstance(v, torch.Tensor) else v)
                if tuple(v.shape) != tuple(t.shape):
                    raise ValueError(f'{k}: shape {tuple(v.shape)} != {tuple(t.shape)}')
                t.copy_(v.to(t.device, torch.float32))

    def get_gradient_dict(self):
        return self.store.named_gradients()

    def early_gradient_range(self):
        self.allocate()
        if self.raw_output:
            return None
        names = list(self.store._entries)
        i0 = names.index('dec.Wr')
        early = {'dec.Wr', f'/{self.name}/att_to_readout.b'}
        early |= {f'/{self.name}/h{l}_to_readout.b' for l in range(1, self.num_layers + 1)}
        for wn, bn, _ in self._out_names:
            early |= {wn, bn}
        i1 = i0
        while i1 < len(names) and names[i1] in early:
            i1 += 1
        lo = self.store.offsets[names[i0]][0]
        o, n = self.store.offsets[names[i1 - 1]]
        return lo, o + (n + 3) // 4 * 4

    @property
    def flat_parameters(self):
        return self.allocate().store.flat

    @property
    def flat_gradients(self):
        return self.allocate().store.flat_grad

    def zero_grad(self):
        self.store.zero_grad()

    def _p(self, short):
        return self.store.param(f'/{self.name}{short}')

    def _g(self, short):
        return self.store.grad(f'/{self.name}{short}')

    def symbolic_input_variables(self):
        speaker = 'speaker_index' if self.use_speaker else None
        raw = 'raw_audio' if self.raw_output else None
        return 'features', 'features_mask', 'labels', 'labels_mask', speaker, 'start_flag', raw

    def initial_states(self, batch_size):
        dev = self._dev()
        f = dict(device=dev, dtype=torch.float32)
        out = []
        carry = self._get_carry(batch_size)
        for l in range(1, 4):
            if l <= self.num_layers:
                out += [self._p(f'/rnn{l}.initial_state').unsqueeze(0).expand(batch_size, -1), carry['h'][l - 1]]
            else:
                out += [None, None]
        out += [self._p('.initial_w').unsqueeze(0).expand(batch_size, -1), carry['w'],
                torch.zeros(batch_size, self.attention_size, **f), carry['k']]
        return tuple(out)

    def _get_carry(self, B):
        c = self._carry.get(B)
        if c is None:
            f = dict(device=self._dev(), dtype=torch.float32)
            c = dict(h=[torch.zeros(B, self.rnn_h_dim, **f) for _ in range(self.num_layers)],
                     c=[torch.zeros(B, self.rnn_h_dim, **f) for _ in range(self.num_layers)],
                     w=torch.zeros(B, self.encoded_input_dim, **f),
                     k=torch.zeros(B, self.attention_size, **f))
            self._carry[B] = c
        return c

    def _samplernn_carry(self, B):
        c = self._carry.get(('srn', B))
        if c is None:
            c = self.sampleRnn.initial_states(B)
            self._carry[('srn', B)] = c
        return c

    def apply_updates(self, updates):
        with torch.no_grad():
            for dst, src in updates:
                dst.copy_(src)

    def _encoder_dims(self, B, U):
        return (B, U) if self.encoder_literal else (U, B)

    def _enc_runner(self, B, U):
        key = ('enc', B, U)
        ws = self._train_ws.get(key)
        if ws is None:
            Te, Be = self._encoder_dims(B, U)
            run = ops.GruSeqRunner(Te, Be, self.encoder_dim, 2, [0, 1], self._dev(), use_graph=self.use_graph)
            ws = dict(run=run)
            self._train_ws[key] = ws
        return ws

    def _encoder_forward(self, labels, labels_mask, save):
        if self.encoder_type is None:
            ctx = labels.to(torch.float32) * labels_mask[..., None]
            return ctx.contiguous()
        B, U = labels.shape
        P = '/encoder/encoder'
        emb = self._p('/encoder/embed_label.W')[labels.long()]
        x = emb if self.encoder_literal else emb.transpose(0, 1)
        x = x.contiguous()
        Te, Be, D = x.shape
        ws = self._enc_runner(B, U)
        run = ws['run']
        x2 = x.reshape(Te * Be, D)
        Wg, Wc = [], []
        for i, d in enumerate(('forward', 'backward')):
            ops.gemm(x2, self._p(f'{P}/{d}/fork/fork_inputs.W'), bias=self._p(f'{P}/{d}/fork/fork_inputs.b'),
                     out=run.inputs[i].view(Te * Be, -1))
            ops.gemm(x2, self._p(f'{P}/{d}/fork/fork_gate_inputs.W'),
                     bias=self._p(f'{P}/{d}/fork/fork_gate_inputs.b'), out=run.gate_inputs[i].view(Te * Be, -1))
            run.h[i][0].copy_(self._p(f'{P}/{d}/gatedrecurrent.initial_state').unsqueeze(0).expand(Be, -1))
            Wg.append(self._p(f'{P}/{d}/gatedrecurrent.state_to_gates'))
            Wc.append(self._p(f'{P}/{d}/gatedrecurrent.state_to_state'))
        run.bind(Wg, Wc)
        run.forward()
        out = torch.cat([run.h[0][1:], run.h[1][1:].flip(0)], dim=-1)
        if not self.encoder_literal:
            out = out.transpose(0, 1)
        ctx = (out * labels_mask[..., None]).contiguous()
        if save is not None:
            save.update(enc_x2=x2, enc_labels=labels, enc_mask=labels_mask)
        return ctx

    def _encoder_backward(self, dctx, save):
        if self.encoder_type is None:
            return
        labels, mask, x2 = save['enc_labels'], save['enc_mask'], save['enc_x2']
        B, U = labels.shape
        P = '/encoder/encoder'
        ED = self.encoder_dim
        run = self._enc_runner(B, U)['run']
        Te, Be = run.T, run.B
        d_out = dctx * mask[..., None]
        if not self.encoder_literal:
            d_out = d_out.transpose(0, 1)
        for i in range(2):
            run.dh[i].zero_()
        run.dh[0][1:].copy_(d_out[..., :ED])
        run.dh[1][1:].copy_(d_out[..., ED:].flip(0))
        run.backward()
        dx = torch.zeros_like(x2)
        for i, d in enumerate(('forward', 'backward')):
            dC = run.dC[i].view(Te * Be, ED)
            dG = run.dG[i].view(Te * Be, 2 * ED)
            hprev = run.h[i][:Te] if i == 0 else run.h[i][:Te].flip(0)
            hprev = hprev.reshape(Te * Be, ED)
            ops.gemm(x2.t(), dC, out=self._g(f'{P}/{d}/fork/fork_inputs.W'), accumulate=True)
            ops.gemm(x2.t(), dG, out=self._g(f'{P}/{d}/fork/fork_gate_inputs.W'), accumulate=True)
            ops.colsum(dC, out=self._g(f'{P}/{d}/fork/fork_inputs.b'), accumulate=True)
            ops.colsum(dG, out=self._g(f'{P}/{d}/fork/fork_gate_inputs.b'), accumulate=True)
            ops.gemm(run.rh[i].view(Te * Be, ED).t(), dC,
                     out=self._g(f'{P}/{d}/gatedrecurrent.state_to_state'), accumulate=True)
            ops.gemm(hprev.t(), dG, out=self._g(f'{P}/{d}/gatedrecurrent.state_to_gates'), accumulate=True)
            ops.colsum(run.dh[i][0], out=self._g(f'{P}/{d}/gatedrecurrent.initial_state'), accumulate=True)
            ops.gemm(dC, self._p(f'{P}/{d}/fork/fork_inputs.W').t(), out=dx, accumulate=True)
            ops.gemm(dG, self._p(f'{P}/{d}/fork/fork_gate_inputs.W').t(), out=dx, accumulate=True)
        demb = dx.view(Te, Be, -1)
        if not self.encoder_literal:
            demb = demb.transpose(0, 1)
        self._scatter_rows_add(self._g('/encoder/embed_label.W'), labels.long().reshape(-1),
                               demb.reshape(-1, demb.shape[-1]))

    def _train_workspace(self, T, B, U):
        ws_key = ('dec', T, B, U)
        ws = self._train_ws.get(ws_key)
        if ws is not None:
            return ws
        H, E, A, L, R = self.rnn_h_dim, self.encoded_input_dim, self.attention_size, self.num_layers, self.readouts_dim
        f = dict(device=self._dev(), dtype=torch.float32)
        ws = dict(
            h=[torch.zeros(T + 1, B, H, **f) for _ in range(L)],
            w=torch.zeros(T + 1, B, E, **f), kappa=torch.zeros(T + 1, B, A, **f),
            a=torch.empty(T, B, A, **f), b=torch.empty(T, B, A, **f), phi=torch.empty(T, B, U, **f),
            dh=[torch.zeros(T + 1, B, H, **f) for _ in range(L)], dw=torch.zeros(T + 1, B, E, **f),
            dw0=torch.zeros(T + 1, B, E, **f),
            dhup=[torch.zeros(T + 1, B, H, **f) if l < L - 1 else None for l in range(L)],
            dkappa=torch.zeros(B, A, **f),
            dp=torch.empty(T, B, 3 * A, **f),
            ctx=torch.zeros(B, U, E, **f),
        )
        lstm = self.cell_type == 'lstm'
        if lstm:
            ws.update(cst=[torch.zeros(T + 1, B, H, **f) for _ in range(L)],
                      gate4=[torch.empty(T, B, 4 * H, **f) for _ in range(L)],
                      dcell=[torch.zeros(B, H, **f) for _ in range(L)])
            if self.compute_bf16 and B <= 64 and H % 32 == 0:
                ws.update(dh_b=[torch.zeros(T + 1, B, H, **f) for _ in range(L)],
                          dhup_b=[torch.zeros(T + 1, B, H, **f) if l < L - 1 else None for l in range(L)],
                          dw_b=torch.zeros(T + 1, B, E, **f), dw0_b=torch.zeros(T + 1, B, E, **f))
        else:
            for n in ('z', 'r', 'rh', 'c'):
                ws[n] = [torch.empty(T, B, H, **f) for _ in range(L)]
        for key, wd, suf, mat, rec in self._groups:
            ws['d' + key.upper()] = [torch.empty(T, B, wd, **f) for _ in range(L)]
            ws['b' + key] = [torch.zeros(wd, **f) for _ in range(L)]
            ws['seq_' + key] = [torch.zeros(T, B, wd, **f) if (l in self._fb_layers or self.use_speaker or l >= 2)
                                else None for l in range(1, L + 1)]
        if (not lstm and L in (2, 3) and not self.compute_bf16 and not self.layer_norm and B <= 64 and H % 16 == 0 and E % 16 == 0
                and env_int('PARROT_BWD_HETERO', 1) != 0):
            ws.update(dh_b=[torch.zeros(T + 1, B, H, **f) for _ in range(L)],
                      dhup_b=[torch.zeros(T + 1, B, H, **f) if l < L - 1 else None for l in range(L)],
                      dhup_c=[torch.zeros(T + 1, B, H, **f) if l < L - 1 else None for l in range(L)],
                      dw_b=torch.zeros(T + 1, B, E, **f), dw0_b=torch.zeros(T + 1, B, E, **f),
                      dw_c=torch.zeros(T + 1, B, E, **f), dw0_c=torch.zeros(T + 1, B, E, **f))
        ln = self.layer_norm and L >= 2
        if ln:
            for key, wd, suf, mat, rec in self._groups:
                ws['ln_y' + key] = {(l, j): torch.empty(T, B, wd, **f) for l in range(1, L) for j in range(l)}
                ws['ln_s' + key] = {(l, j): torch.empty(T, B, **f) for l in range(1, L) for j in range(l)}
        d = _lib.DecoderDesc()
        d.cell = 1 if lstm else 0
        d.layer_norm = 1 if ln else 0
        d.bf16 = 1 if self.compute_bf16 else 0
        if ln:
            for key, wd, suf, mat, rec in self._groups:
                for (l, j), t_ in ws['ln_y' + key].items():
                    pj = l * _lib.MAX_LAYERS + j
                    getattr(d, 'ln_y' + key)[pj] = t_.data_ptr()
                    getattr(d, 'ln_s' + key)[pj] = ws['ln_s' + key][(l, j)].data_ptr()
                    getattr(d, 'ln_b' + key)[pj] = self._p(f'/h{j + 1}_to_h{l + 1}/fork_rnn{l + 1}_{suf}.b').data_ptr()
        d.seq_init = sum(1 << (l - 1) for l in range(1, L + 1) if (l in self._fb_layers or self.use_speaker))
        d.T, d.B, d.H, d.E, d.A, d.U, d.L = T, B, H, E, A, U, L
        d.att_type = 1 if self.attention_type == 'softmax' else 0
        d.use_graph = int(self.use_graph)
        d.reserved = 0
        d.eps, d.alignment, d.sharpening, d.timing = self.epsilon, self.attention_alignment, 1.0, 1.0
        st = self.store.storage
        for l in range(L):
            for key, wd, suf, mat, rec in self._groups:
                getattr(d, 'W' + key)[l] = st[f'{mat}{l + 1}'].data_ptr()
                getattr(d, 'b' + key)[l] = ws['b' + key][l].data_ptr()
                sq = ws['seq_' + key][l]
                getattr(d, 'seq_' + key)[l] = sq.data_ptr() if sq is not None else None
                getattr(d, 'd' + key.upper())[l] = ws['d' + key.upper()][l].data_ptr()
            for n in (('h', 'dh', 'cst', 'gate4', 'dcell') if lstm else ('h', 'dh', 'z', 'r', 'rh', 'c')):
                getattr(d, n)[l] = ws[n][l].data_ptr()
            d.dhup[l] = ws['dhup'][l].data_ptr() if ws['dhup'][l] is not None else None
            if 'dh_b' in ws:
                d.dh_b[l] = ws['dh_b'][l].data_ptr()
                d.dhup_b[l] = ws['dhup_b'][l].data_ptr() if ws['dhup_b'][l] is not None else None
                if 'dhup_c' in ws:
                    d.dhup_c[l] = ws['dhup_c'][l].data_ptr() if ws['dhup_c'][l] is not None else None
        tl = self._tiled_weights()
        if tl is not None:
            for l in range(L):
                for key, wd, suf, mat, rec in self._groups:
                    getattr(d, f'W{key}_f')[l] = tl[(l, key, 'f')].data_ptr()
                    getattr(d, f'W{key}_r')[l] = tl[(l, key, 'r')].data_ptr()
        ws['att_sup'] = torch.zeros(T, B, 2, device=self._dev(), dtype=torch.int32)
        d.att_sup = ws['att_sup'].data_ptr()
        if env_int('PARROT_SCHEDULE', -1) == 4 and tl is not None:
            n = int(_lib.load().parrot_decoder_persist_floats(C.byref(d)))
            if n > 0:
                ws['persist_ws'] = torch.zeros(n, **f)
                d.persist_ws, d.persist_ws_floats = ws['persist_ws'].data_ptr(), n
        d.WattT, d.batt, d.ctx = st['dec.WattT'].data_ptr(), st['dec.batt'].data_ptr(), ws['ctx'].data_ptr()
        for n in ('w', 'kappa', 'a', 'b', 'phi', 'dw', 'dw0', 'dkappa', 'dp'):
            setattr(d, n, ws[n].data_ptr())
        if 'dw_b' in ws:
            d.dw_b, d.dw0_b = ws['dw_b'].data_ptr(), ws['dw0_b'].data_ptr()
        if 'dw_c' in ws:
            d.dw_c, d.dw0_c = ws['dw_c'].data_ptr(), ws['dw0_c'].data_ptr()
        if lstm and self._bf16_weight_grads(0, T, T) and env_int('PARROT_BF16_DG16', 1) != 0:
            cp = self._bf16_copies(ws, T, B)
            for l in range(L):
                d.dG16[l] = cp['d']['g'][l].data_ptr()
        plan = C.c_void_p()
        _lib.call('parrot_decoder_create', C.byref(d), C.byref(plan))
        ws['plan'], ws['desc'] = plan, d
        ws['plan_writes_d16'] = bool(_lib.load().parrot_decoder_writes_bf16_grads(plan))
        self._train_ws[ws_key] = ws
        return ws

    @staticmethod
    def _scatter_rows_add(grad, idx, src):
        onehot = torch.zeros(idx.numel(), grad.shape[0], device=grad.device, dtype=torch.float32)
        onehot.scatter_(1, idx.reshape(-1, 1), 1.0)
        with ops.gemm_precision(ops.PRECISION_F32):
            ops.gemm(onehot.t(), src.contiguous(), out=grad, accumulate=True)

    def _tiled_weights(self, refresh=False):
        H, E = self.rnn_h_dim, self.encoded_input_dim
        bf = self.compute_bf16
        if bf and (H % 32 or E % 32 or self.layer_norm):
            raise ValueError("compute_dtype='bf16' needs rnn_h_dim and the encoder width to be multiples of 32 "
                             "and layer_norm=False")
        if H % 16 or E % 16:
            return None
        if getattr(self, '_tiled', None) is None:
            st = self.store.storage
            self._tiled = {}
            for l in range(self.num_layers):
                for key, wd, suf, mat, rec in self._groups:
                    for which in ('f', 'r'):
                        self._tiled[(l, key, which)] = torch.empty_like(
                            st[f'{mat}{l + 1}'], dtype=torch.bfloat16 if bf else torch.float32)
            refresh = True
        if refresh:
            st = self.store.storage
            for l in range(self.num_layers):
                for key, wd, suf, mat, rec in self._groups:
                    W = st[f'{mat}{l + 1}']
                    lstm_h = H if self.cell_type == 'lstm' else 0
                    fn = 'parrot_tile_weights_bf16' if bf else 'parrot_tile_weights'
                    _lib.call(fn, W.data_ptr(), W.shape[0], W.shape[1], W.shape[1],
                              self._tiled[(l, key, 'f')].data_ptr(), 0, lstm_h, ops._stream())
                    _lib.call(fn, W.data_ptr(), W.shape[0], W.shape[1], W.shape[1],
                              self._tiled[(l, key, 'r')].data_ptr(), 1, 0, ops._stream())
        return self._tiled

    def _layer_bias_names(self, l, suf):
        names = [f'/inp_to_h{l}/fork_rnn{l}_{suf}.b']
        if not self.layer_norm:
            names += [f'/h{j}_to_h{l}/fork_rnn{l}_{suf}.b' for j in range(1, l)]
        return names

    def _sum_layer_biases(self, ws, extra_fb=False):
        for l in range(1, self.num_layers + 1):
            for key, wd, suf, mat, rec in self._groups:
                b = ws['b' + key][l - 1]
                b.zero_()
                for n in self._layer_bias_names(l, suf):
                    b.add_(self._p(n))
                if extra_fb and l in self._fb_layers:
                    b.add_(self._p(f'/out_to_h{l}/fork_rnn{l}_{suf}.b'))

    def compute_cost(self, *args, **kwargs):
        with ops.gemm_precision(ops.PRECISION_BF16 if self.compute_bf16 else ops.full_precision()):
            return self._compute_cost(*args, **kwargs)

    def _backward(self, token, gscale):
        with ops.gemm_precision(ops.PRECISION_BF16 if self.compute_bf16 else ops.full_precision()):
            return self._backward_f(token, gscale)

    def _compute_cost(self, features, features_mask, labels, labels_mask, speaker, start_flag,
                      batch_size, raw_audio=None, feedback_noise=None):
        self.allocate()
        if speaker is None:
            assert not self.use_speaker
        if self.raw_output and raw_audio is None:
            raise ValueError("raw_output=True needs the raw_audio source (datasets.py:194-203)")
        dev = self._dev()
        features = features.to(dev, torch.float32)
        features_mask = features_mask.to(dev, torch.float32)
        labels_mask = labels_mask.to(dev, torch.float32)
        labels = labels.to(dev)
        target = features[1:]
        mask = features_mask[1:].contiguous()
        T, B = mask.shape
        assert B == batch_size
        U = labels.shape[1]
        H, E, L, R, O = self.rnn_h_dim, self.encoded_input_dim, self.num_layers, self.readouts_dim, self.output_dim
        ws = self._train_workspace(T, B, U)
        save = dict(T=T, B=B, U=U, ws=ws, start_flag=int(bool(start_flag)))

        inp = None
        if self.weak_feedback:
            inp = features[:-1]
            if self.feedback_noise_level:
                if feedback_noise is None:
                    feedback_noise = self.feedback_noise_level * torch.randn_like(inp)
                inp = inp + feedback_noise
            inp = inp.reshape(T * B, O).contiguous()
            save['fb_inp'] = inp
        emb_spk = None
        if self.use_speaker:
            emb_spk = self._p('/lookuptable.W')[speaker[:, 0].long()].contiguous()
            save['spk_idx'], save['emb_spk'] = speaker[:, 0].long(), emb_spk
        for l in range(1, L + 1):
            for key, wd, suf, mat, rec in self._groups:
                sq = ws['seq_' + key][l - 1]
                if sq is None or not (l in self._fb_layers or self.use_speaker):
                    continue
                have = False
                if l in self._fb_layers:
                    if self.layer_norm:
                        y, sig = ops.simple_norm_fwd(
                            ops.gemm(inp, self._p(f'/out_to_h{l}/fork_rnn{l}_{suf}.W'),
                                     bias=self._p(f'/out_to_h{l}/fork_rnn{l}_{suf}.b')))
                        save[('ln_fb', l, key)] = (y, sig)
                        sq.view(T * B, wd).copy_(y)
                    else:
                        ops.gemm(inp, self._p(f'/out_to_h{l}/fork_rnn{l}_{suf}.W'),
                                 bias=self._p(f'/out_to_h{l}/fork_rnn{l}_{suf}.b'), out=sq.view(T * B, wd))
                    have = True
                if self.use_speaker:
                    sp = ops.gemm(emb_spk, self._p(f'/speaker_to_h{l}/fork_rnn{l}_{suf}.W'),
                                  bias=self._p(f'/speaker_to_h{l}/fork_rnn{l}_{suf}.b'))
                    if self.layer_norm:
                        sp, sig = ops.simple_norm_fwd(sp)
                        save[('ln_spk', l, key)] = (sp, sig)
                    if have:
                        sq.add_(sp.unsqueeze(0))
                    else:
                        sq.copy_(sp.unsqueeze(0).expand(T, -1, -1))

        carry = self._get_carry(B)
        for l in range(L):
            if start_flag:
                ws['h'][l][0].copy_(self._p(f'/rnn{l + 1}.initial_state').unsqueeze(0).expand(B, -1))
            else:
                ws['h'][l][0].copy_(carry['h'][l])
            if self.cell_type == 'lstm':
                if start_flag:
                    ws['cst'][l][0].copy_(self._p(f'/rnn{l + 1}.initial_cells').unsqueeze(0).expand(B, -1))
                else:
                    ws['cst'][l][0].copy_(carry['c'][l])
        if start_flag:
            ws['w'][0].copy_(self._p('.initial_w').unsqueeze(0).expand(B, -1))
            ws['kappa'][0].zero_()
        else:
            ws['w'][0].copy_(carry['w'])
            ws['kappa'][0].copy_(carry['k'])

        with ops.gemm_precision(ops.PRECISION_F32):
            ws['ctx'].copy_(self._encoder_forward(labels, labels_mask, save))
        self._sum_layer_biases(ws)
        self._tiled_weights(refresh=True)

        _lib.call('parrot_decoder_seq_fwd', ws['plan'], ops._stream())
        if 'persist_ws' in ws:
            _lib.call('parrot_decoder_status', ws['plan'])

        composed = save['readout_composed'] = self._readout_composed()
        self._readout_path = 'composed' if composed else 'factored'
        if composed:
            rd = self._readout_desc(ws, T, B)
            pr = torch.empty(T * B, O, device=dev, dtype=torch.float32)
            rd.pred = pr.data_ptr()
            _lib.call('parrot_readout_composed_fwd', C.byref(rd), ws['ro_ws'].data_ptr(), ops._stream())
            preds = [pr.view(T, B, O)]
        else:
            preds = self._readouts_factored(ws, save, T, B, emb_spk)

        gmm_fused = self._gmm_cost_fused()
        self._gmm_cost_path = None if self.which_cost != 'GMM' else ('fused' if gmm_fused else 'torch')
        leafs = [] if gmm_fused else [p.detach().requires_grad_(True) for p in preds]
        with torch.enable_grad():
            if gmm_fused:
                M = T * B
                tgt, heads = target.reshape(M, O), [p.view(M, -1) for p in preds]
                nll, pi, logr = ops.gmm_cost_fwd(tgt, *heads, self.epsilon)
                mrow, msum = mask.view(M), mask.sum() + 1e-5
                cost_val = (nll * mrow).sum() / msum
                save['gmm'] = (tgt, heads, logr, mrow / msum)
                next_x, coeff = preds[0], pi.view(T, B, self.k_gmm)
            elif self.which_cost == 'MSE':
                cost_tb = ((leafs[0] - target) ** 2).sum(-1)
                next_x, coeff = preds[0], preds[0]
            else:
                sigma = torch.exp(leafs[1]) + self.epsilon
                coeff_ = torch.softmax(leafs[2], -1) + self.epsilon
                cost_tb = cost_gmm(target, leafs[0], sigma, coeff_)
                next_x, coeff = preds[0], coeff_.detach()
            if not gmm_fused:
                cost_val = (cost_tb * mask).sum() / (mask.sum() + 1e-5)
        cost_raw = None
        if self.raw_output:
            tt = self.sampleRnn.three_tier
            raw = torch.as_tensor(raw_audio).to(dev)
            raw_mask = features_mask.repeat_interleave(80, dim=0).t().contiguous()
            raw_seq = raw.permute(1, 0, 2).reshape(B, -1).long()
            last_h0, last_big_h0 = self._samplernn_carry(B)
            with torch.enable_grad():
# ... 774 lines not shown
```

### parrot_amd/ops.py

```python
from __future__ import annotations

import torch

from . import _lib
from .utils import env_int, env_str

ACT_NONE, ACT_RELU, ACT_TANH, ACT_SIGMOID = 0, 1, 2, 3


def _stream() -> int:
    return torch.cuda.current_stream().cuda_stream


def _chk(t: torch.Tensor, name: str, dtype=torch.float32):
    if not isinstance(t, torch.Tensor) or not t.is_cuda:
        raise _lib.HipCallError(
            f"{name}: the parrot_amd product path needs a GPU tensor (got {type(t).__name__}"
            f"{'' if not isinstance(t, torch.Tensor) else ' on ' + str(t.device)}); there is no CPU fallback")
    if t.dtype != dtype:
        raise TypeError(f"{name}: expected {dtype}, got {t.dtype}")


def ptr(t, name="tensor", dtype=torch.float32) -> int:
    if t is None:
# ... 24 lines not shown
        raise ValueError("gemm: accumulate together with an activation is not defined")
    pa, M, K, lda, ta = _mat(a, "a")
    pb, K2, N, ldb, tb = _mat(b, "b")
    if K != K2:
        raise ValueError(f"gemm: inner dimensions differ ({K} vs {K2})")
    if out is None:
        if accumulate:
            out = torch.zeros((M, N), device=a.device, dtype=torch.float32)
        else:
            out = torch.empty((M, N), device=a.device, dtype=torch.float32)
    _chk(out, "out")
    if out.shape != (M, N) or out.stride(1) != 1:
        raise ValueError("gemm: bad output tensor")
    if M == 0 or N == 0:
        return out
    if K == 0:
        if not accumulate:
            out.zero_()
        return out
    _lib.call("parrot_gemm", pa, lda, ta, pb, ldb, tb, out.data_ptr(), out.stride(0), M, N, K,
              ptr(bias, "bias"), float(alpha), int(bool(accumulate)), int(act), 1, 0, 0, 0, int(split_k),
              _stream())
    return out


ROUTE_STEP, ROUTE_F32, ROUTE_BF16, ROUTE_BF16X3 = 0, 1, 2, 3


def gemm_route(a: torch.Tensor, b: torch.Tensor, bias=None, out=None, accumulate=False, act=ACT_NONE, alpha=1.0,
               split_k=0, gate=None, nbatch=None, transA=False, transB=False):
    import ctypes as C
    if nbatch is not None:
        _chk(a, "a"); _chk(b, "b")
        if a.shape[0] != nbatch or b.shape[0] != nbatch:
            raise ValueError("gemm_route: nbatch does not match the operands")
        M, K = (a.shape[2], a.shape[1]) if transA else (a.shape[1], a.shape[2])
        N = b.shape[1] if transB else b.shape[2]
        args = (a.data_ptr(), a.stride(1), int(transA), b.data_ptr(), b.stride(1), int(transB), M, N, K, 1.0, 0,
                int(nbatch), a.stride(0), b.stride(0), 1, 0)
    else:
        pa, M, K, lda, ta = _mat(a, "a")
        pb, K2, N, ldb, tb = _mat(b, "b")
        if K != K2:
            raise ValueError(f"gemm_route: inner dimensions differ ({K} vs {K2})")
        if gate is not None:
            args = (pa, lda, ta, pb, ldb, tb, M, N, K, 1.0, 0, 1, 0, 0, 0, 1)
        else:
            args = (pa, lda, ta, pb, ldb, tb, M, N, K, float(alpha), int(act), 1, 0, 0, int(split_k), 0)
    kernel, slices = C.c_int(-1), C.c_int(-1)
    _lib.call("parrot_gemm_route", *args, C.byref(kernel), C.byref(slices))
    return kernel.value, slices.value


def to_bf16(x: torch.Tensor, out=None) -> torch.Tensor:
    _chk(x, "x")
    if not x.is_contiguous() or x.numel() % 8:
        raise ValueError("to_bf16: contiguous tensor with a multiple of 8 elements expected")
    if out is None:
        out = torch.empty(x.shape, device=x.device, dtype=torch.bfloat16)
    if out.dtype != torch.bfloat16 or out.numel() != x.numel() or not out.is_contiguous() or not out.is_cuda:
        raise ValueError("to_bf16: bad output tensor")
    _lib.call("parrot_to_bf16", x.data_ptr(), out.data_ptr(), x.numel(), _stream())
    return out


def gemm_bf16in(a_t: torch.Tensor, b: torch.Tensor, out: torch.Tensor, accumulate=False, split_k=0) -> torch.Tensor:
    for x_, n_ in ((a_t, "a_t"), (b, "b")):
        if not (x_.is_cuda and x_.dtype == torch.bfloat16 and x_.dim() == 2 and x_.stride(1) == 1):
            raise ValueError(f"gemm_bf16in: {n_} must be a 2-d bf16 GPU tensor with unit inner stride")
    _chk(out, "out")
    K, M = a_t.shape
    K2, N = b.shape
    if K != K2 or out.shape != (M, N) or out.stride(1) != 1:
        raise ValueError("gemm_bf16in: shapes do not match")
    _lib.call("parrot_gemm_bf16in", a_t.data_ptr(), a_t.stride(0), b.data_ptr(), b.stride(0), out.data_ptr(),
              out.stride(0), M, N, K, int(bool(accumulate)), int(split_k), _stream())
    return out


def gemm16(a: torch.Tensor, b: torch.Tensor, out=None, bias=None, accumulate=False, split_k=0) -> torch.Tensor:
    pa, M, K, lda, ta = _mat16(a, "a")
    pb, K2, N, ldb, tb = _mat16(b, "b")
    if K != K2:
        raise ValueError(f"gemm16: inner dimensions differ ({K} vs {K2})")
    if out is None:
        out = (torch.zeros if accumulate else torch.empty)((M, N), device=a.device, dtype=torch.float32)
    _chk(out, "out")
    if out.shape != (M, N) or out.stride(1) != 1:
        raise ValueError("gemm16: bad output tensor")
    _lib.call("parrot_gemm_bf16in_ex", pa, lda, ta, pb, ldb, tb, out.data_ptr(), out.stride(0), M, N, K,
              ptr(bias, "bias"), int(bool(accumulate)), int(split_k), _stream())
    return out


def _mat16(t: torch.Tensor, name: str):
    _chk(t, name, torch.bfloat16)
    if t.dim() != 2:
        raise ValueError(f"{name}: expected a 2-D tensor")
    if t.stride(1) == 1 and t.stride(0) >= max(1, t.shape[1]):
        return t.data_ptr(), t.shape[0], t.shape[1], t.stride(0), 0
    if t.stride(0) == 1 and t.stride(1) >= max(1, t.shape[0]):
        return t.data_ptr(), t.shape[0], t.shape[1], t.stride(1), 1
    raise ValueError(f"{name}: unsupported strides {t.stride()}")


PRECISION_F32, PRECISION_BF16, PRECISION_BF16X3 = 0, 1, 2


def _default_full_precision() -> int:
    return PRECISION_F32 if env_str("PARROT_GEMM_PRECISION", "") in ("f32", "0") else PRECISION_BF16X3


_FULL_PRECISION = _default_full_precision()


def full_precision() -> int:
    return _FULL_PRECISION


def set_full_precision(mode: int) -> int:
    global _FULL_PRECISION
    if mode not in (PRECISION_F32, PRECISION_BF16X3):
        raise ValueError("set_full_precision: PRECISION_F32 or PRECISION_BF16X3")
    prev, _FULL_PRECISION = _FULL_PRECISION, int(mode)
    _lib.call("parrot_set_gemm_precision", int(mode))
    return prev


class gemm_precision:

    def __init__(self, mode):
        self.mode = int(mode)

    def __enter__(self):
        self.prev = int(_lib.load().parrot_get_gemm_precision())
        _lib.call("parrot_set_gemm_precision", self.mode)
        return self

    def __exit__(self, *exc):
        _lib.call("parrot_set_gemm_precision", self.prev)
        return False


def gemm_batched(a, b, out, transA=False, transB=False, accumulate=False):
    _chk(a, "a"); _chk(b, "b"); _chk(out, "out")
    nb = a.shape[0]
    M, K = (a.shape[2], a.shape[1]) if transA else (a.shape[1], a.shape[2])
    N = b.shape[1] if transB else b.shape[2]
    assert a.stride(2) == 1 and b.stride(2) == 1 and out.stride(2) == 1
    _lib.call("parrot_gemm", a.data_ptr(), a.stride(1), int(transA), b.data_ptr(), b.stride(1), int(transB),
              out.data_ptr(), out.stride(1), M, N, K, None, 1.0, int(bool(accumulate)), 0, nb,
              a.stride(0), b.stride(0), out.stride(0), 1, _stream())
    return out


def colsum(x: torch.Tensor, out=None, accumulate=False) -> torch.Tensor:
    _chk(x, "x")
    x2 = x.reshape(-1, x.shape[-1])
    if x2.stride(1) != 1:
        x2 = x2.contiguous()
    M, N = x2.shape
    if out is None:
        out = torch.empty((N,), device=x.device, dtype=torch.float32)
        accumulate = False
    if M == 0:
        if not accumulate:
            out.zero_()
        return out
    _lib.call("parrot_colsum", x2.data_ptr(), M, N, x2.stride(0), out.data_ptr(), int(bool(accumulate)), _stream())
    return out


class _LinearFn(torch.autograd.Function):

    @staticmethod
    def forward(ctx, x, W, b, act):
        x2 = x.reshape(-1, x.shape[-1])
        if x2.stride(-1) != 1:
            x2 = x2.contiguous()
        y = gemm(x2, W, bias=b, act=act)
        ctx.save_for_backward(x2, W, y if act != ACT_NONE else None)
        ctx.act = act
        ctx.has_b = b is not None
        ctx.xshape = x.shape
        return y.reshape(*x.shape[:-1], W.shape[1])

    @staticmethod
    def backward(ctx, dy):
        x2, W, y = ctx.saved_tensors
        dy2 = dy.reshape(-1, dy.shape[-1])
        if ctx.act == ACT_RELU:
            dy2 = dy2 * (y > 0).to(dy2.dtype)
        elif ctx.act == ACT_TANH:
            dy2 = dy2 * (1 - y * y)
        elif ctx.act == ACT_SIGMOID:
            dy2 = dy2 * y * (1 - y)
        if not dy2.is_contiguous():
            dy2 = dy2.contiguous()
        dx = dW = db = None
        if ctx.needs_input_grad[0]:
            dx = gemm(dy2, W.t()).reshape(ctx.xshape)
        if ctx.needs_input_grad[1]:
            dW = gemm(x2.t(), dy2)
        if ctx.has_b and ctx.needs_input_grad[2]:
            db = colsum(dy2)
        return dx, dW, db, None


def linear(x, W, b=None, act=ACT_NONE):
    return _LinearFn.apply(x, W, b, act)


def gemm_gated(a: torch.Tensor, b: torch.Tensor, gate: torch.Tensor, out=None) -> torch.Tensor:
    pa, M, K, lda, ta = _mat(a, "a")
    pb, K2, N, ldb, tb = _mat(b, "b")
    _chk(gate, "gate")
    if K != K2 or gate.shape != (M, N) or gate.stride(1) != 1:
        raise ValueError("gemm_gated: shapes do not match")
    if out is None:
        out = torch.empty((M, N), device=a.device, dtype=torch.float32)
    _chk(out, "out")
    if out.shape != (M, N) or out.stride(1) != 1:
        raise ValueError("gemm_gated: bad output tensor")
    _lib.call("parrot_gemm_gated", pa, lda, ta, pb, ldb, tb, out.data_ptr(), out.stride(0), M, N, K,
              gate.data_ptr(), gate.stride(0), _stream())
    return out


def _int32(t: torch.Tensor, name: str, bound=None) -> torch.Tensor:
    if not isinstance(t, torch.Tensor) or not t.is_cuda:
        raise _lib.HipCallError(f"{name}: the parrot_amd product path needs a GPU tensor; there is no CPU fallback")
    t32 = t.to(torch.int32).contiguous()
    if bound is not None and t32.numel() and not _SKIP_INDEX_CHECK:
        lo, hi = int(t32.min()), int(t32.max())
        if lo < 0 or hi >= bound:
            raise IndexError(f"{name}: values in [{lo}, {hi}] outside [0, {bound})")
    return t32


_SKIP_INDEX_CHECK = env_int("PARROT_SKIP_INDEX_CHECK", 0) != 0


class _EmbedSumFn(torch.autograd.Function):

    @staticmethod
    def forward(ctx, E, W1, idx, add):
        Q, EMB = E.shape
        N, J = idx.shape
        D = W1.shape[1]
        if W1.shape[0] != J * EMB:
            raise ValueError("embed_sum: W1 must be [J * EMB, D]")
        E_, W1_ = E.contiguous(), W1.contiguous()
        idx32 = _int32(idx, "idx", bound=Q)
        tbl = torch.empty(J, Q, D, device=E.device, dtype=torch.float32)
        with gemm_precision(PRECISION_F32):
            gemm_batched(E_.unsqueeze(0).expand(J, -1, -1), W1_.view(J, EMB, D), tbl)
        y = torch.empty(N, D, device=E.device, dtype=torch.float32)
        if add is not None:
            _chk(add, "add")
            add = add.reshape(N, D)
            if add.stride(1) != 1:
                add = add.contiguous()
        _lib.call("parrot_gather_sum_fwd", tbl.data_ptr(), idx32.data_ptr(), add.data_ptr() if add is not None else None,
                  add.stride(0) if add is not None else 0, y.data_ptr(), y.stride(0), N, J, Q, D, _stream())
        ctx.save_for_backward(E_, W1_, idx32)
        ctx.has_add = add is not None
        return y

    @staticmethod
    def backward(ctx, dy):
        E, W1, idx32 = ctx.saved_tensors
        Q, EMB = E.shape
        N, J = idx32.shape
        D = W1.shape[1]
        dy = dy.reshape(N, D)
        if dy.stride(1) != 1:
            dy = dy.contiguous()
        vals, perm = torch.sort(idx32.t().contiguous(), dim=1, stable=True)
        bins = torch.arange(Q + 1, device=E.device, dtype=torch.int32).unsqueeze(0).expand(J, -1).contiguous()
        offs = torch.searchsorted(vals, bins).to(torch.int32).contiguous()
        perm = perm.to(torch.int32).contiguous()
        n_ws = int(_lib.load().parrot_gather_sum_bwd_ws_floats(N, J, Q, D))
        ws = torch.empty(n_ws, device=E.device, dtype=torch.float32)
        dtbl = torch.empty(J, Q, D, device=E.device, dtype=torch.float32)
        _lib.call("parrot_gather_sum_bwd", dy.data_ptr(), dy.stride(0), perm.data_ptr(), offs.data_ptr(), dtbl.data_ptr(),
                  ws.data_ptr(), n_ws, N, J, Q, D, 0, _stream())
        dE = dW1 = None
        with gemm_precision(PRECISION_F32):
            if ctx.needs_input_grad[0]:
                t = torch.empty(J, Q, EMB, device=E.device, dtype=torch.float32)
                gemm_batched(dtbl, W1.view(J, EMB, D), t, transB=True)
                dE = t.sum(0)
            if ctx.needs_input_grad[1]:
                dW1 = torch.empty(J, EMB, D, device=E.device, dtype=torch.float32)
                gemm_batched(E.unsqueeze(0).expand(J, -1, -1), dtbl, dW1, transA=True)
                dW1 = dW1.view(J * EMB, D)
        return dE, dW1, None, (dy if ctx.has_add and ctx.needs_input_grad[3] else None)


def embed_sum(E, W1, idx, add=None):
    return _EmbedSumFn.apply(E, W1, idx, add)


class _ReluMlpFn(torch.autograd.Function):

    @staticmethod
    def forward(ctx, x, W2, b2, W3, b3, W4, b4):
        x = x.reshape(-1, x.shape[-1])
        if x.stride(1) != 1:
            x = x.contiguous()
        y2 = gemm(x, W2, bias=b2, act=ACT_RELU)
        y3 = gemm(y2, W3, bias=b3, act=ACT_RELU)
        out = gemm(y3, W4, bias=b4)
        ctx.save_for_backward(x, y2, y3, W2, W3, W4)
        return out

    @staticmethod
    def backward(ctx, dl):
        x, y2, y3, W2, W3, W4 = ctx.saved_tensors
        if not dl.is_contiguous():
            dl = dl.contiguous()
        need = ctx.needs_input_grad
        d3 = gemm_gated(dl, W4.t(), y3)
        dW4 = gemm(y3.t(), dl) if need[5] else None
        db4 = colsum(dl) if need[6] else None
        d2 = gemm_gated(d3, W3.t(), y2)
        dW3 = gemm(y2.t(), d3) if need[3] else None
        db3 = colsum(d3) if need[4] else None
        dW2 = gemm(x.t(), d2) if need[1] else None
        db2 = colsum(d2) if need[2] else None
        dx = gemm(d2, W2.t()) if need[0] else None
        return dx, dW2, db2, dW3, db3, dW4, db4


def relu_mlp(x, W2, b2, W3, b3, W4, b4):
    return _ReluMlpFn.apply(x, W2, b2, W3, b3, W4, b4)


class _SoftmaxCeFn(torch.autograd.Function):

    @staticmethod
    def forward(ctx, logits, target):
        _chk(logits, "logits")
        x = logits.reshape(-1, logits.shape[-1])
        if x.stride(1) != 1:
            x = x.contiguous()
        rows, Q = x.shape
        t32 = _int32(target.reshape(-1), "target", bound=Q)
        if t32.numel() != rows:
            raise ValueError("softmax_ce: one target per row expected")
        lse = torch.empty(rows, device=x.device, dtype=torch.float32)
        ce = torch.empty(rows, device=x.device, dtype=torch.float32)
        _lib.call("parrot_softmax_ce_fwd", x.data_ptr(), x.stride(0), t32.data_ptr(), rows, Q, lse.data_ptr(),
                  ce.data_ptr(), _stream())
        ctx.save_for_backward(x, t32, lse)
        ctx.lshape = logits.shape
        return ce

    @staticmethod
    def backward(ctx, g):
        x, t32, lse = ctx.saved_tensors
        rows, Q = x.shape
        g = g.reshape(-1).to(torch.float32).contiguous()
        dx = torch.empty(rows, Q, device=x.device, dtype=torch.float32)
        _lib.call("parrot_softmax_ce_bwd", x.data_ptr(), x.stride(0), t32.data_ptr(), lse.data_ptr(), g.data_ptr(), rows, Q,
                  dx.data_ptr(), dx.stride(0), _stream())
        return dx.view(ctx.lshape), None


def softmax_ce(logits, target):
    return _SoftmaxCeFn.apply(logits, target)


def _gmm_rows(y, mu, sig_hat, co_hat):
    for t, n in ((y, "y"), (mu, "mu"), (sig_hat, "sig_hat"), (co_hat, "co_hat")):
        _chk(t, n)
        if t.dim() != 2 or t.stride(1) != 1:
            raise ValueError(f"gmm_cost: {n} must be 2-D with unit column stride")
    (M, O), K = y.shape, co_hat.shape[1]
    if M < 1 or O < 1 or K < 1:
        raise ValueError("gmm_cost: empty operand")
    if mu.shape != (M, O * K) or sig_hat.shape != (M, O * K) or co_hat.shape[0] != M:
        raise ValueError(f"gmm_cost: y [M, O], mu / sig_hat [M, O*K], co_hat [M, K] expected, got {tuple(y.shape)}, "
                         f"{tuple(mu.shape)}, {tuple(sig_hat.shape)}, {tuple(co_hat.shape)}")
    return M, O, K


def _ld(t):
    return t.stride(0) if t.shape[0] > 1 else max(t.stride(0), t.shape[1])


def gmm_cost_fwd(y, mu, sig_hat, co_hat, eps, pi_out=None):
    M, O, K = _gmm_rows(y, mu, sig_hat, co_hat)
    nll = torch.empty(M, device=y.device, dtype=torch.float32)
    logr = torch.empty(M, K, device=y.device, dtype=torch.float32)
    if pi_out is None:
        pi_out = torch.empty(M, K, device=y.device, dtype=torch.float32)
    _chk(pi_out, "pi_out")
    if pi_out.shape != (M, K) or pi_out.stride(1) != 1:
        raise ValueError("gmm_cost_fwd: pi_out must be [M, K] with unit column stride")
    _lib.call("parrot_gmm_cost_fwd", y.data_ptr(), _ld(y), mu.data_ptr(), _ld(mu), sig_hat.data_ptr(), _ld(sig_hat),
              co_hat.data_ptr(), _ld(co_hat), M, O, K, float(eps), nll.data_ptr(), pi_out.data_ptr(), _ld(pi_out),
              logr.data_ptr(), _stream())
    return nll, pi_out, logr


def gmm_cost_bwd(y, mu, sig_hat, co_hat, logr, rowscale, eps, out=None):
    M, O, K = _gmm_rows(y, mu, sig_hat, co_hat)
    _chk(logr, "logr"); _chk(rowscale, "rowscale")
    if logr.shape != (M, K) or not logr.is_contiguous():
        raise ValueError("gmm_cost_bwd: logr must be the contiguous [M, K] array of gmm_cost_fwd")
    if rowscale.numel() != M or not rowscale.is_contiguous():
        raise ValueError("gmm_cost_bwd: one rowscale per row expected")
    if out is None:
        out = (torch.empty(M, O * K, device=y.device, dtype=torch.float32),
               torch.empty(M, O * K, device=y.device, dtype=torch.float32),
               torch.empty(M, K, device=y.device, dtype=torch.float32))
    dmu, dsig, dco = out
    for t, n, w in ((dmu, "dmu", O * K), (dsig, "dsig_hat", O * K), (dco, "dco_hat", K)):
        _chk(t, n)
        if t.shape != (M, w) or t.stride(1) != 1:
            raise ValueError(f"gmm_cost_bwd: {n} must be [M, {w}] with unit column stride")
    _lib.call("parrot_gmm_cost_bwd", y.data_ptr(), _ld(y), mu.data_ptr(), _ld(mu), sig_hat.data_ptr(), _ld(sig_hat),
              co_hat.data_ptr(), _ld(co_hat), logr.data_ptr(), rowscale.data_ptr(), M, O, K, float(eps),
              dmu.data_ptr(), _ld(dmu), dsig.data_ptr(), _ld(dsig), dco.data_ptr(), _ld(dco), _stream())
    return dmu, dsig, dco


class _GmmNllFn(torch.autograd.Function):

    @staticmethod
    def forward(ctx, y, mu, sig_hat, co_hat, eps):
        nll, _, logr = gmm_cost_fwd(y, mu, sig_hat, co_hat, eps)
        ctx.save_for_backward(y, mu, sig_hat, co_hat, logr)
        ctx.eps = eps
        return nll

    @staticmethod
    def backward(ctx, g):
        y, mu, sig_hat, co_hat, logr = ctx.saved_tensors
        g = g.reshape(-1).to(torch.float32).contiguous()
        dmu, dsig, dco = gmm_cost_bwd(y, mu, sig_hat, co_hat, logr, g, ctx.eps)
        return None, dmu, dsig, dco, None


def gmm_nll(y, mu, sig_hat, co_hat, eps):
    return _GmmNllFn.apply(y, mu, sig_hat, co_hat, eps)


class _WeightNormFn(torch.autograd.Function):

    @staticmethod
    def forward(ctx, W, g):
        _chk(W, "W"); _chk(g, "g")
        if W.dim() != 2 or g.dim() != 1 or g.shape[0] != W.shape[1]:
            raise ValueError("weightnorm_fold: W [K, N], g [N] expected")
        Wc = W if W.stride(1) == 1 else W.contiguous()
        gc = g.contiguous()
        K, N = Wc.shape
        out = torch.empty(K, N, device=W.device, dtype=torch.float32)
        norm = torch.empty(N, device=W.device, dtype=torch.float32)
        ws = torch.empty(int(_lib.load().samplernn_weightnorm_ws_floats(N)), device=W.device, dtype=torch.float32)
        _lib.call("samplernn_weightnorm_fold", Wc.data_ptr(), Wc.stride(0), gc.data_ptr(), out.data_ptr(), N, norm.data_ptr(),
                  ws.data_ptr(), K, N, _stream())
        ctx.save_for_backward(Wc, gc, norm)
        return out

    @staticmethod
    def backward(ctx, d):
        Wc, gc, norm = ctx.saved_tensors
        K, N = Wc.shape
        d = d.to(torch.float32)
        if d.stride(1) != 1:
            d = d.contiguous()
        dW = torch.empty(K, N, device=Wc.device, dtype=torch.float32)
        dg = torch.empty(N, device=Wc.device, dtype=torch.float32)
        ws = torch.empty(int(_lib.load().samplernn_weightnorm_ws_floats(N)), device=Wc.device, dtype=torch.float32)
        _lib.call("samplernn_weightnorm_fold_bwd", Wc.data_ptr(), Wc.stride(0), gc.data_ptr(), norm.data_ptr(), d.data_ptr(),
                  d.stride(0), dW.data_ptr(), N, dg.data_ptr(), ws.data_ptr(), K, N, 0, 0, _stream())
        return dW, dg


def weightnorm_fold(W, g):
    return _WeightNormFn.apply(W, g)


def gru_step_fwd(h, inputs, gate_inputs, Wg, Wc, mask=None):
    B, H = h.shape
    z, r, rh, c, out = (torch.empty((B, H), device=h.device, dtype=torch.float32) for _ in range(5))
    _lib.call("parrot_gru_step_fwd", ptr(h, "h"), ptr(inputs, "inputs"), ptr(gate_inputs, "gate_inputs"),
              ptr(mask, "mask"), ptr(Wg, "Wg"), ptr(Wc, "Wc"), ptr(out), ptr(z), ptr(r), ptr(rh), ptr(c),
              B, H, _stream())
    return out, (z, r, rh, c)


def gru_step_bwd(dh_out, h, Wg, Wc, saved, mask=None):
    z, r, rh, c = saved
    B, H = h.shape
    dh = torch.empty((B, H), device=h.device, dtype=torch.float32)
    dC = torch.empty((B, H), device=h.device, dtype=torch.float32)
    dG = torch.empty((B, 2 * H), device=h.device, dtype=torch.float32)
    _lib.call("parrot_gru_step_bwd", ptr(dh_out, "dh_out"), ptr(h, "h"), ptr(mask, "mask"), ptr(Wg), ptr(Wc),
              ptr(z), ptr(r), ptr(c), ptr(dh), ptr(dC), ptr(dG), B, H, _stream())
    return dh, dC, dG


class _GruStepFn(torch.autograd.Function):
    @staticmethod
    def forward(ctx, inputs, gate_inputs, h, Wc, Wg, mask):
        inputs, gate_inputs, h = inputs.contiguous(), gate_inputs.contiguous(), h.contiguous()
        out, saved = gru_step_fwd(h, inputs, gate_inputs, Wg, Wc, mask)
        ctx.save_for_backward(h, Wc, Wg, mask, *saved)
        return out

    @staticmethod
    def backward(ctx, dout):
        h, Wc, Wg, mask, z, r, rh, c = ctx.saved_tensors
        dh, dC, dG = gru_step_bwd(dout.contiguous(), h, Wg, Wc, (z, r, rh, c), mask)
        dWc = gemm(rh.t(), dC) if ctx.needs_input_grad[3] else None
        dWg = gemm(h.t(), dG) if ctx.needs_input_grad[4] else None
        return dC, dG, dh, dWc, dWg, None


def gru_step(inputs, gate_inputs, h, Wc, Wg, mask=None):
    return _GruStepFn.apply(inputs, gate_inputs, h, Wc, Wg, mask)


class GruSeqRunner:

    def __init__(self, T, B, H, nchain, reverse, device, use_graph=False, with_backward=True):
        import ctypes as C
        self.T, self.B, self.H, self.nchain = T, B, H, nchain
        self.reverse = list(reverse)
        f = dict(device=device, dtype=torch.float32)
        self.h = [torch.zeros((T + 1, B, H), **f) for _ in range(nchain)]
        self.z, self.r, self.rh, self.c = ([torch.empty((T, B, H), **f) for _ in range(nchain)] for _ in range(4))
        self.inputs = [torch.zeros((T, B, H), **f) for _ in range(nchain)]
        self.gate_inputs = [torch.zeros((T, B, 2 * H), **f) for _ in range(nchain)]
        self.mask = None
        self.with_backward = with_backward
        if with_backward:
            self.dh = [torch.zeros((T + 1, B, H), **f) for _ in range(nchain)]
            self.dG = [torch.empty((T, B, 2 * H), **f) for _ in range(nchain)]
            self.dC = [torch.empty((T, B, H), **f) for _ in range(nchain)]
        self.use_graph = use_graph
        self._plan = None
        self._weights = None

    def bind(self, Wg, Wc, mask=None):
        import ctypes as C
        key = tuple(w.data_ptr() for w in list(Wg) + list(Wc)) + ((mask.data_ptr(),) if mask is not None else ())
        if self._plan is not None and key == self._weights:
            return
        self.close()
        d = _lib.GruSeqDesc()
        d.T, d.B, d.H, d.nchain, d.use_graph = self.T, self.B, self.H, self.nchain, int(self.use_graph)
        for i in range(self.nchain):
            d.reverse[i] = int(self.reverse[i])
            d.Wg[i], d.Wc[i] = ptr(Wg[i], "Wg"), ptr(Wc[i], "Wc")
            d.inputs[i], d.gate_inputs[i] = self.inputs[i].data_ptr(), self.gate_inputs[i].data_ptr()
            d.h[i] = self.h[i].data_ptr()
            d.z[i], d.r[i], d.rh[i], d.c[i] = (x[i].data_ptr() for x in (self.z, self.r, self.rh, self.c))
            if self.with_backward:
                d.dh[i], d.dG[i], d.dC[i] = self.dh[i].data_ptr(), self.dG[i].data_ptr(), self.dC[i].data_ptr()
        d.mask = ptr(mask, "mask") if mask is not None else None
        self.mask = mask
        plan = C.c_void_p()
        _lib.call("parrot_gru_seq_create", C.byref(d), C.byref(plan))
        self._plan, self._weights = plan, key
        self._keep = (list(Wg), list(Wc), mask)

    def forward(self):
        _lib.call("parrot_gru_seq_fwd", self._plan, _stream())

    def backward(self):
        _lib.call("parrot_gru_seq_bwd", self._plan, _stream())

    def close(self):
        if self._plan is not None:
            _lib.load().parrot_gru_seq_destroy(self._plan)
            self._plan = None

    def __del__(self):
        try:
            self.close()
        except Exception:
            pass


class _GruSeqFn(torch.autograd.Function):

    @staticmethod
    def forward(ctx, inputs, gate_inputs, h0, Wc, Wg, mask, reverse):
        T, B, H = inputs.shape
        run = GruSeqRunner(T, B, H, 1, [reverse], inputs.device, use_graph=False)
        run.inputs[0].copy_(inputs)
        run.gate_inputs[0].copy_(gate_inputs)
        run.h[0][0].copy_(h0)
        run.bind([Wg], [Wc], mask.contiguous() if mask is not None else None)
        run.forward()
        ctx.run = run
        ctx.reverse = reverse
        ctx.save_for_backward(Wc, Wg)
        hs = run.h[0][1:]
        return hs.flip(0) if reverse else hs.clone()

# ... 172 lines not shown
```

Before: 889,300 frames/s.

## Precompute encoder fork projections per label and add 8-wave row GRU kernels

The encoder input projections are now computed once per vocabulary entry (a Q-row table GEMM) and gathered by label instead of running a GEMM over every token. In backward, gradients are reduced per label with a new double-precision segmented sum, then a small GEMM produces the weight and embedding gradients. Separately, the row-wise GRU kernels are templated on wave count and default to 8 waves, with precomputed prefetch offsets and idle-wave guards. The table path only applies when the vocabulary size is at most 64. It adds workspace and new kernels, and changes floating-point summation order and contraction behaviour.

```diff
diff --git a/include/parrot_hip.h b/include/parrot_hip.h
--- a/include/parrot_hip.h
+++ b/include/parrot_hip.h
@@ -303,6 +303,21 @@
                           long long rows, int Q, float* dlogits, int ldd, void* stream);
 int parrot_relu_gate(const float* dy, const float* gate, float* out, long long n, void* stream);
 
+typedef struct ParrotLabelTablesDesc {
+    long long N;
+    int Q, nseg;
+    const int* labels;
+    const float* tbl[4];
+    float* rows[4];
+    float* sums[4];
+    int D[4];
+} ParrotLabelTablesDesc;
+
+int parrot_label_tables_supported(long long N, int Q);
+int parrot_label_gather(const ParrotLabelTablesDesc* desc, void* stream);
+long long parrot_label_segsum_ws_floats(long long N, int Q, int Dtotal);
+int parrot_label_segsum(const ParrotLabelTablesDesc* desc, float* ws, long long ws_floats, void* stream);
+
 int parrot_gmm_cost_fwd(const float* y, int ldy, const float* mu, int ldmu, const float* sig_hat, int ldsig,
                         const float* co_hat, int ldco, long long M, int O, int K, float eps, float* nll, float* pi_out,
                         int ldpi, float* logr, void* stream);
diff --git a/parrot_amd/_lib.py b/parrot_amd/_lib.py
--- a/parrot_amd/_lib.py
+++ b/parrot_amd/_lib.py
@@ -32,6 +32,15 @@
         ("h", C.c_void_p * 4),
         ("z", C.c_void_p * 4), ("r", C.c_void_p * 4), ("rh", C.c_void_p * 4), ("c", C.c_void_p * 4),
         ("dh", C.c_void_p * 4), ("dG", C.c_void_p * 4), ("dC", C.c_void_p * 4),
+    ]
+
+
+class LabelTablesDesc(C.Structure):
+    _fields_ = [
+        ("N", C.c_longlong), ("Q", C.c_int), ("nseg", C.c_int),
+        ("labels", C.c_void_p),
+        ("tbl", C.c_void_p * 4), ("rows", C.c_void_p * 4), ("sums", C.c_void_p * 4),
+        ("D", C.c_int * 4),
     ]
 
 
@@ -178,6 +187,10 @@
     "parrot_colsum": (_i, [_vp, _ll, _i, _i, _vp, _i, _vp]),
     "parrot_gru_step_fwd": (_i, [_vp] * 11 + [_i, _i, _vp]),
     "parrot_gru_step_bwd": (_i, [_vp] * 11 + [_i, _i, _vp]),
+    "parrot_label_tables_supported": (_i, [_ll, _i]),
+    "parrot_label_gather": (_i, [C.POINTER(LabelTablesDesc), _vp]),
+    "parrot_label_segsum_ws_floats": (C.c_longlong, [_ll, _i, _i]),
+    "parrot_label_segsum": (_i, [C.POINTER(LabelTablesDesc), _vp, _ll, _vp]),
     "parrot_gru_seq_create": (_i, [C.POINTER(GruSeqDesc), C.POINTER(C.c_void_p)]),
     "parrot_gru_seq_fwd": (_i, [_vp, _vp]),
     "parrot_gru_seq_bwd": (_i, [_vp, _vp]),
diff --git a/parrot_amd/build.py b/parrot_amd/build.py
--- a/parrot_amd/build.py
+++ b/parrot_amd/build.py
@@ -16,7 +16,7 @@
 
 SOURCES = ["skinny.hip", "biggemm.hip", "attention.hip", "elementwise.hip", "quantize.hip",
            "plans.hip", "plans_decode.hip", "capi.hip", "samplernn.hip", "persist.hip", "sr_persist.hip", "rowgru.hip", "trainops.hip", "readout.hip",
-           "gmmcost.hip"]
+           "gmmcost.hip", "labeltables.hip"]
 EXTRA_FLAGS = {"quantize.hip": ["-ffp-contract=off"]}
 if env_str("PARROT_PM_DEPTH"):
     EXTRA_FLAGS["persist.hip"] = ["-DPM_DEPTH=" + env_str("PARROT_PM_DEPTH")]
diff --git a/parrot_amd/csrc/labeltables.hip b/parrot_amd/csrc/labeltables.hip
--- /dev/null
+++ b/parrot_amd/csrc/labeltables.hip
@@ -0,0 +1,162 @@
+#include <stdlib.h>
+
+#include "../../include/parrot_hip.h"
+#include "common.h"
+
+namespace {
+
+constexpr int LT_MAXQ = 64;
+constexpr int LT_WAVES = 2, LT_THREADS = 64 * LT_WAVES;
+constexpr int LT_RPS = 128;
+
+struct LtArgs {
+    const int* labels;
+    const float* tbl[4];
+    float* rows[4];
+    float* sums[4];
+    int D[4], c0[5];
+    long long N;
+    int Q, nseg;
+};
+
+__global__ __launch_bounds__(256) void lt_gather_kernel(const LtArgs a) {
+    const int G = a.c0[a.nseg] >> 2;
+    const long long e = (long long)blockIdx.x * 256 + threadIdx.x;
+    if (e >= a.N * G) return;
+    const long long i = e / G;
+    const int col = 4 * (int)(e % G);
+    const int q = min(max(a.labels[i], 0), a.Q - 1);
+#pragma unroll
+    for (int s = 0; s < 4; ++s)
+        if (s < a.nseg && col >= a.c0[s] && col < a.c0[s + 1]) {
+            const int c = col - a.c0[s];
+            *reinterpret_cast<f32x4*>(a.rows[s] + (size_t)i * a.D[s] + c) =
+                *reinterpret_cast<const f32x4*>(a.tbl[s] + (size_t)q * a.D[s] + c);
+        }
+}
+
+__device__ __forceinline__ const float* lt_column(const LtArgs& a, int col, int& pitch) {
+    const float* p = nullptr;
+    pitch = 0;
+#pragma unroll
+    for (int s = 0; s < 4; ++s)
+        if (s < a.nseg && col >= a.c0[s] && col < a.c0[s + 1]) {
+            p = a.rows[s] + (col - a.c0[s]);
+            pitch = a.D[s];
+        }
+    return p;
+}
+
+__global__ __launch_bounds__(LT_THREADS) void lt_segsum_slice_kernel(const LtArgs a, double* __restrict__ ws) {
+    extern __shared__ double tab[];
+    const int lane = threadIdx.x & 63, wave = threadIdx.x >> 6;
+    const int Q = a.Q, Dt = a.c0[a.nseg];
+    const int col = blockIdx.y * 64 + lane;
+    double* mine = tab + (size_t)wave * Q * 64;
+    for (int q = 0; q < Q; ++q) mine[q * 64 + lane] = 0.0;
+    int pitch;
+    const float* src = lt_column(a, col, pitch);
+    const long long r0 = (long long)blockIdx.x * LT_RPS, r1 = min(a.N, r0 + LT_RPS);
+    if (src) {
+        long long r = r0 + wave;
+        for (; r + 3 * LT_WAVES < r1; r += 4 * LT_WAVES) {
+            float v[4];
+            int q[4];
+#pragma unroll
+            for (int u = 0; u < 4; ++u) {
+                v[u] = src[(size_t)(r + LT_WAVES * u) * pitch];
+                q[u] = min(max(a.labels[r + LT_WAVES * u], 0), Q - 1);
+            }
+#pragma unroll
+            for (int u = 0; u < 4; ++u) mine[q[u] * 64 + lane] += (double)v[u];
+        }
+        for (; r < r1; r += LT_WAVES) mine[min(max(a.labels[r], 0), Q - 1) * 64 + lane] += (double)src[(size_t)r * pitch];
+    }
+    __syncthreads();
+    if (col < Dt)
+        for (int q = wave; q < Q; q += LT_WAVES) {
+            double t = 0.0;
+#pragma unroll
+            for (int w = 0; w < LT_WAVES; ++w) t += tab[((size_t)w * Q + q) * 64 + lane];
+            ws[((size_t)blockIdx.x * Q + q) * Dt + col] = t;
+        }
+}
+
+__global__ __launch_bounds__(256) void lt_segsum_reduce_kernel(const LtArgs a, const double* __restrict__ ws, int nslices) {
+    const int Q = a.Q, Dt = a.c0[a.nseg];
+    const int q = blockIdx.x, col = blockIdx.y * 256 + threadIdx.x;
+    if (col >= Dt) return;
+    const double* p = ws + (size_t)q * Dt + col;
+    const size_t step = (size_t)Q * Dt;
+    double acc = 0.0;
+    int sl = 0;
+    for (; sl + 8 <= nslices; sl += 8) {
+        double v[8];
+#pragma unroll
+        for (int u = 0; u < 8; ++u) v[u] = p[(size_t)(sl + u) * step];
+#pragma unroll
+        for (int u = 0; u < 8; ++u) acc += v[u];
+    }
+    for (; sl < nslices; ++sl) acc += p[(size_t)sl * step];
+    const float out = (float)acc;
+#pragma unroll
+    for (int s = 0; s < 4; ++s)
+        if (s < a.nseg && col >= a.c0[s] && col < a.c0[s + 1]) a.sums[s][(size_t)q * a.D[s] + (col - a.c0[s])] = out;
+}
+
+int lt_args(const ParrotLabelTablesDesc* d, bool gather, LtArgs& a) {
+    if (!d || !d->labels || d->N < 1 || d->Q < 1 || d->nseg < 1 || d->nseg > 4) return PH_ERR_BADARG;
+    if (d->Q > LT_MAXQ) return PH_ERR_UNSUPPORTED;
+    a.labels = d->labels; a.N = d->N; a.Q = d->Q; a.nseg = d->nseg;
+    a.c0[0] = 0;
+    for (int s = 0; s < 4; ++s) {
+        a.tbl[s] = nullptr; a.rows[s] = nullptr; a.sums[s] = nullptr; a.D[s] = 0;
+        if (s >= d->nseg) { a.c0[s + 1] = a.c0[s]; continue; }
+        if (d->D[s] < 4 || (d->D[s] & 3) || !d->rows[s] || !(gather ? (const void*)d->tbl[s] : (const void*)d->sums[s]))
+            return PH_ERR_BADARG;
+        if (((uintptr_t)d->rows[s] & 15) || (gather && ((uintptr_t)d->tbl[s] & 15))) return PH_ERR_BADARG;
+        a.tbl[s] = d->tbl[s]; a.rows[s] = d->rows[s]; a.sums[s] = d->sums[s]; a.D[s] = d->D[s];
+        a.c0[s + 1] = a.c0[s] + d->D[s];
+    }
+    return 0;
+}
+
+}
+
+extern "C" {
+
+int parrot_label_tables_supported(long long N, int Q) { return N >= 1 && Q >= 1 && Q <= LT_MAXQ; }
+
+int parrot_label_gather(const ParrotLabelTablesDesc* desc, void* stream) { PH_ENTRY();
+    LtArgs a;
+    const int rc = lt_args(desc, true, a);
+    if (rc) return rc;
+    const long long blocks = (a.N * (a.c0[a.nseg] >> 2) + 255) / 256;
+    if (blocks > 0x7fffffffll) return PH_ERR_UNSUPPORTED;
+    hipLaunchKernelGGL(lt_gather_kernel, dim3((unsigned)blocks), dim3(256), 0, (hipStream_t)stream, a);
+    return (int)hipGetLastError();
+}
+
+long long parrot_label_segsum_ws_floats(long long N, int Q, int Dtotal) { PH_ENTRY();
+    if (N < 1 || Q < 1 || Dtotal < 1) return 0;
+    return 2 * ((N + LT_RPS - 1) / LT_RPS) * Q * Dtotal;
+}
+
+int parrot_label_segsum(const ParrotLabelTablesDesc* desc, float* ws, long long ws_floats, void* stream) { PH_ENTRY();
+    LtArgs a;
+    const int rc = lt_args(desc, false, a);
+    if (rc) return rc;
+    const int Dt = a.c0[a.nseg];
+    if (!ws || ((uintptr_t)ws & 7) || ws_floats < parrot_label_segsum_ws_floats(a.N, a.Q, Dt)) return PH_ERR_BADARG;
+    const long long nslices = (a.N + LT_RPS - 1) / LT_RPS;
+    if (nslices > 0x7fffffffll) return PH_ERR_UNSUPPORTED;
+    double* wsd = reinterpret_cast<double*>(ws);
+    hipLaunchKernelGGL(lt_segsum_slice_kernel, dim3((unsigned)nslices, (unsigned)ceil_div(Dt, 64)), dim3(LT_THREADS),
+                       sizeof(double) * LT_WAVES * a.Q * 64, (hipStream_t)stream, a, wsd);
+    PH_CHECK(hipGetLastError());
+    hipLaunchKernelGGL(lt_segsum_reduce_kernel, dim3((unsigned)a.Q, (unsigned)ceil_div(Dt, 256)), dim3(256), 0,
+                       (hipStream_t)stream, a, wsd, (int)nslices);
+    return (int)hipGetLastError();
+}
+
+}
diff --git a/parrot_amd/csrc/plans.hip b/parrot_amd/csrc/plans.hip
--- a/parrot_amd/csrc/plans.hip
+++ b/parrot_amd/csrc/plans.hip
@@ -7,6 +7,7 @@
     ParrotGruSeqDesc d;
 
     bool rowwise = false;
+    int waves = 4;
     float* tiled = nullptr;
     ~GruSeqPlan() override {
         if (tiled) (void)hipFree(tiled);
@@ -16,6 +17,7 @@
         for (int ch = 0; ch < d.nchain && rowwise; ++ch)
             if (!d.Wg[ch] || !d.Wc[ch] || ((uintptr_t)d.Wg[ch] & 15) || ((uintptr_t)d.Wc[ch] & 15)) rowwise = false;
         if (!rowwise) return 0;
+        waves = rowgru_waves(sw_rg_waves());
         const size_t per = (size_t)6 * d.H * d.H;
         if (hipMalloc(&tiled, sizeof(float) * per * d.nchain) != hipSuccess) {
             tiled = nullptr;
@@ -36,7 +38,7 @@
             c.dh = d.dh[ch]; c.dG = d.dG[ch]; c.dC = d.dC[ch];
             c.reverse = d.reverse[ch];
         }
-        g.mask = d.mask; g.T = d.T; g.B = d.B; g.H = d.H; g.nchain = d.nchain;
+        g.mask = d.mask; g.T = d.T; g.B = d.B; g.H = d.H; g.nchain = d.nchain; g.waves = waves;
         return g;
     }
     int fwd_rowwise(hipStream_t st) {
diff --git a/parrot_amd/csrc/rowgru.h b/parrot_amd/csrc/rowgru.h
--- a/parrot_amd/csrc/rowgru.h
+++ b/parrot_amd/csrc/rowgru.h
@@ -17,8 +17,10 @@
     RowGruChain chain[4];
     const float* mask;
     int T, B, H, nchain;
+    int waves;
 };
 
 bool rowgru_supported(int T, int B, int H, int nchain);
+int rowgru_waves(int requested);
 int rowgru_fwd_launch(const RowGruArgs& g, hipStream_t stream);
 int rowgru_bwd_launch(const RowGruArgs& g, hipStream_t stream);
diff --git a/parrot_amd/csrc/rowgru.hip b/parrot_amd/csrc/rowgru.hip
--- a/parrot_amd/csrc/rowgru.hip
+++ b/parrot_amd/csrc/rowgru.hip
@@ -2,17 +2,19 @@
 
 #include "skinny.h"
 
+#pragma clang fp contract(off)
+
 namespace {
 
-constexpr int RG_THREADS = 256, RG_ROWS = 16, RG_MAXH = 128;
+constexpr int RG_ROWS = 16, RG_MAXH = 128;
 
 __device__ __forceinline__ float rg_sigmoid(float x) { return 1.0f / (1.0f + expf(-x)); }
 
-template <int NT, int NCH>
+template <int NW, int NT, int NCH>
 __device__ __forceinline__ void rg_load_w(const float* __restrict__ Bt, int ct0, int ntiles, int lane, f32x4 (&wb)[NT][NCH]) {
 #pragma unroll
     for (int q = 0; q < NT; ++q) {
-        const int ct = min(ct0 + 4 * q, ntiles - 1);
+        const int ct = min(ct0 + NW * q, ntiles - 1);
 #pragma unroll
         for (int c = 0; c < NCH; ++c) wb[q][c] = *reinterpret_cast<const f32x4*>(Bt + ((size_t)ct * NCH + c) * 256 + 4 * lane);
     }
@@ -32,9 +34,10 @@
     }
 }
 
-template <int NCH>
-__global__ __launch_bounds__(RG_THREADS) void rg_fwd_kernel(const RowGruArgs g) {
-    constexpr int NTG = (2 * NCH + 3) / 4, NTC = (NCH + 3) / 4;
+template <int NCH, int NW>
+__global__ __launch_bounds__(64 * NW) void rg_fwd_kernel(const RowGruArgs g) {
+    constexpr int THREADS = 64 * NW;
+    constexpr int NTG = (2 * NCH + NW - 1) / NW, NTC = (NCH + NW - 1) / NW;
     extern __shared__ __attribute__((aligned(16))) float sm[];
     const int H = g.H, B = g.B, T = g.T, P = H + 4;
     float* s_h = sm;
@@ -45,33 +48,42 @@
     const RowGruChain& c = g.chain[ch];
     const size_t BH = (size_t)B * H;
     const int ntg = (2 * H) >> 4, ntc = H >> 4;
+    const bool g_wave = wave < ntg, c_wave = wave < ntc;
     f32x4 wg[NTG][NCH], wc[NTC][NCH];
-    rg_load_w<NTG, NCH>(c.Wg_f, wave, ntg, lane, wg);
-    rg_load_w<NTC, NCH>(c.Wc_f, wave, ntc, lane, wc);
-    for (int e = tid; e < RG_ROWS * H; e += RG_THREADS) {
+    if (g_wave) rg_load_w<NW, NTG, NCH>(c.Wg_f, wave, ntg, lane, wg);
+    if (c_wave) rg_load_w<NW, NTC, NCH>(c.Wc_f, wave, ntc, lane, wc);
+    for (int e = tid; e < RG_ROWS * H; e += THREADS) {
         const int m = e / H, k = e % H;
         s_h[m * P + k] = (m0 + m < B) ? c.h[(size_t)(m0 + m) * H + k] : 0.f;
     }
     __syncthreads();
     const int gq = lane >> 4, jj = lane & 15;
-    float pg[NTG][4], pc[NTC][4];
+    float pg[NTG][4] = {}, pc[NTC][4] = {};
+    unsigned og[NTG][4], oc[NTC][4];
+#pragma unroll
+    for (int r = 0; r < 4; ++r) {
+        const unsigned mr = min(m0 + 4 * gq + r, B - 1);
+#pragma unroll
+        for (int q = 0; q < NTG; ++q) og[q][r] = mr * 2 * H + 16 * min(wave + NW * q, ntg - 1) + jj;
+#pragma unroll
+        for (int q = 0; q < NTC; ++q) oc[q][r] = mr * H + 16 * min(wave + NW * q, ntc - 1) + jj;
+    }
     auto prefetch = [&](int s) {
         const int t = c.reverse ? T - 1 - s : s;
-#pragma unroll
-        for (int q = 0; q < NTG; ++q)
-#pragma unroll
-            for (int r = 0; r < 4; ++r) {
-                const int n = 16 * (wave + 4 * q) + jj, mr = m0 + 4 * gq + r;
-                pg[q][r] = (c.gate_inputs && s < T && wave + 4 * q < ntg && mr < B)
-                               ? c.gate_inputs[(size_t)t * 2 * BH + (size_t)mr * 2 * H + n] : 0.f;
-            }
-#pragma unroll
-        for (int q = 0; q < NTC; ++q)
-#pragma unroll
-            for (int r = 0; r < 4; ++r) {
-                const int n = 16 * (wave + 4 * q) + jj, mr = m0 + 4 * gq + r;
-                pc[q][r] = (c.inputs && s < T && wave + 4 * q < ntc && mr < B) ? c.inputs[(size_t)t * BH + (size_t)mr * H + n] : 0.f;
-            }
+        if (c.gate_inputs && g_wave) {
+            const float* src = c.gate_inputs + (size_t)t * 2 * BH;
+#pragma unroll
+            for (int q = 0; q < NTG; ++q)
+#pragma unroll
+                for (int r = 0; r < 4; ++r) pg[q][r] = src[og[q][r]];
+        }
+        if (c.inputs && c_wave) {
+            const float* src = c.inputs + (size_t)t * BH;
+#pragma unroll
+            for (int q = 0; q < NTC; ++q)
+#pragma unroll
+                for (int r = 0; r < 4; ++r) pc[q][r] = src[oc[q][r]];
+        }
     };
     prefetch(0);
     for (int s = 0; s < T; ++s) {
@@ -85,13 +97,13 @@
         for (int q = 0; q < NTC; ++q)
 #pragma unroll
             for (int r = 0; r < 4; ++r) cc_in[q][r] = pc[q][r];
-        prefetch(s + 1);
-        {
+        if (s + 1 < T) prefetch(s + 1);
+        if (g_wave) {
             f32x4 acc[NTG];
             rg_mma<NTG, NCH>(s_h, P, wg, lane, acc);
 #pragma unroll
             for (int q = 0; q < NTG; ++q) {
-                const int ct = wave + 4 * q;
+                const int ct = wave + NW * q;
                 if (ct >= ntg) continue;
                 const int n = 16 * ct + jj;
 #pragma unroll
@@ -114,12 +126,12 @@
             }
         }
         __syncthreads();
-        {
+        if (c_wave) {
             f32x4 acc[NTC];
             rg_mma<NTC, NCH>(s_rh, P, wc, lane, acc);
 #pragma unroll
             for (int q = 0; q < NTC; ++q) {
-                const int ct = wave + 4 * q;
+                const int ct = wave + NW * q;
                 if (ct >= ntc) continue;
                 const int n = 16 * ct + jj;
 #pragma unroll
@@ -129,10 +141,10 @@
                     const float pre = acc[q][r] + cc_in[q][r];
                     const float cc = tanhf(pre);
                     const float z = s_z[m * P + n], hp = s_h[m * P + n];
-                    float hn = z * cc + (1.f - z) * hp;
+                    float hn = fmaf(z, cc, (1.f - z) * hp);
                     if (g.mask) {
                         const float mk = g.mask[(size_t)t * B + mr];
-                        hn = mk * hn + (1.f - mk) * hp;
+                        hn = fmaf(mk, hn, (1.f - mk) * hp);
                     }
                     c.c[(size_t)t * BH + (size_t)mr * H + n] = cc;
                     c.h[(size_t)(s + 1) * BH + (size_t)mr * H + n] = hn;
@@ -144,9 +156,12 @@
     }
 }
 
-template <int NCH>
-__global__ __launch_bounds__(RG_THREADS) void rg_bwd_kernel(const RowGruArgs g) {
-    constexpr int NTC = (NCH + 3) / 4;
+template <int NCH, int NW>
+__global__ __launch_bounds__(64 * NW) void rg_bwd_kernel(const RowGruArgs g) {
+    constexpr int THREADS = 64 * NW;
+    constexpr int NTC = (NCH + NW - 1) / NW;
+    constexpr int NE = (4 * NCH + NW - 1) / NW;
+    constexpr bool EVEN = (4 * NCH) % NW == 0;
     extern __shared__ __attribute__((aligned(16))) float sm[];
     const int H = g.H, B = g.B, T = g.T, P = H + 4, P2 = 2 * H + 4;
     float* s_cur = sm;
@@ -158,52 +173,68 @@
     const RowGruChain& c = g.chain[ch];
     const size_t BH = (size_t)B * H;
     const int ntc = H >> 4;
+    const bool t_wave = wave < ntc;
     f32x4 wx[NTC][NCH], wy[NTC][2 * NCH];
-    rg_load_w<NTC, NCH>(c.Wc_r, wave, ntc, lane, wx);
-    rg_load_w<NTC, 2 * NCH>(c.Wg_r, wave, ntc, lane, wy);
-    for (int e = tid; e < RG_ROWS * H; e += RG_THREADS) {
+    if (t_wave) {
+        rg_load_w<NW, NTC, NCH>(c.Wc_r, wave, ntc, lane, wx);
+        rg_load_w<NW, NTC, 2 * NCH>(c.Wg_r, wave, ntc, lane, wy);
+    }
+    for (int e = tid; e < RG_ROWS * H; e += THREADS) {
         const int m = e / H, k = e % H;
         s_cur[m * P + k] = (m0 + m < B) ? c.dh[(size_t)T * BH + (size_t)(m0 + m) * H + k] : 0.f;
     }
     __syncthreads();
     const int gq = lane >> 4, jj = lane & 15;
-    float p_hp[NCH], p_z[NCH], p_c[NCH], p_r[NTC][4], p_hp2[NTC][4], p_slot[NTC][4];
+    float p_hp[NE], p_z[NE], p_c[NE], p_r[NTC][4], p_hp2[NTC][4], p_slot[NTC][4];
+    unsigned oe[NE], ot[NTC][4];
+#pragma unroll
+    for (int i = 0; i < NE; ++i) {
+        const int e = min(tid + THREADS * i, RG_ROWS * H - 1);
+        oe[i] = (unsigned)min(m0 + e / H, B - 1) * H + e % H;
+    }
+#pragma unroll
+    for (int q = 0; q < NTC; ++q)
+#pragma unroll
+        for (int r = 0; r < 4; ++r) ot[q][r] = (unsigned)min(m0 + 4 * gq + r, B - 1) * H + 16 * min(wave + NW * q, ntc - 1) + jj;
     auto prefetch = [&](int s) {
         const int t = c.reverse ? T - 1 - s : s;
-#pragma unroll
-        for (int i = 0; i < NCH; ++i) {
-            const int e = tid + RG_THREADS * i, m = e / H, k = e % H, mr = m0 + m;
-            const bool ok = s >= 0 && mr < B;
-            const size_t ix = ok ? (size_t)t * BH + (size_t)mr * H + k : 0;
-            p_hp[i] = ok ? c.h[(size_t)s * BH + (size_t)mr * H + k] : 0.f;
-            p_z[i] = ok ? c.z[ix] : 0.f;
-            p_c[i] = ok ? c.c[ix] : 0.f;
-        }
-#pragma unroll
-        for (int q = 0; q < NTC; ++q)
-#pragma unroll
-            for (int r = 0; r < 4; ++r) {
-                const int n = 16 * (wave + 4 * q) + jj, mr = m0 + 4 * gq + r;
-                const bool ok = s >= 0 && wave + 4 * q < ntc && mr < B;
-                p_r[q][r] = ok ? c.r[(size_t)t * BH + (size_t)mr * H + n] : 0.f;
-                p_hp2[q][r] = ok ? c.h[(size_t)s * BH + (size_t)mr * H + n] : 0.f;
-                p_slot[q][r] = ok ? c.dh[(size_t)s * BH + (size_t)mr * H + n] : 0.f;
-            }
+        const float* hs = c.h + (size_t)s * BH;
+        const float* zt = c.z + (size_t)t * BH;
+        const float* ct = c.c + (size_t)t * BH;
+#pragma unroll
+        for (int i = 0; i < NE; ++i) {
+            p_hp[i] = hs[oe[i]];
+            p_z[i] = zt[oe[i]];
+            p_c[i] = ct[oe[i]];
+        }
+        if (t_wave) {
+            const float* rt = c.r + (size_t)t * BH;
+            const float* ds = c.dh + (size_t)s * BH;
+#pragma unroll
+            for (int q = 0; q < NTC; ++q)
+#pragma unroll
+                for (int r = 0; r < 4; ++r) {
+                    p_r[q][r] = rt[ot[q][r]];
+                    p_hp2[q][r] = hs[ot[q][r]];
+                    p_slot[q][r] = ds[ot[q][r]];
+                }
+        }
     };
     prefetch(T - 1);
     for (int s = T - 1; s >= 0; --s) {
         const int t = c.reverse ? T - 1 - s : s;
-        float q_hp[NCH], q_z[NCH], q_c[NCH], q_r[NTC][4], q_hp2[NTC][4], q_slot[NTC][4];
-#pragma unroll
-        for (int i = 0; i < NCH; ++i) { q_hp[i] = p_hp[i]; q_z[i] = p_z[i]; q_c[i] = p_c[i]; }
+        float q_hp[NE], q_z[NE], q_c[NE], q_r[NTC][4], q_hp2[NTC][4], q_slot[NTC][4];
+#pragma unroll
+        for (int i = 0; i < NE; ++i) { q_hp[i] = p_hp[i]; q_z[i] = p_z[i]; q_c[i] = p_c[i]; }
 #pragma unroll
         for (int q = 0; q < NTC; ++q)
 #pragma unroll
             for (int r = 0; r < 4; ++r) { q_r[q][r] = p_r[q][r]; q_hp2[q][r] = p_hp2[q][r]; q_slot[q][r] = p_slot[q][r]; }
-        prefetch(s - 1);
-#pragma unroll
-        for (int ei = 0; ei < NCH; ++ei) {
-            const int e = tid + RG_THREADS * ei;
+        if (s > 0) prefetch(s - 1);
+#pragma unroll
+        for (int ei = 0; ei < NE; ++ei) {
+            const int e = tid + THREADS * ei;
+            if (!EVEN && e >= RG_ROWS * H) continue;
             const int m = e / H, k = e % H, mr = m0 + m;
             float dC = 0.f, dGz = 0.f, dhp = 0.f;
             if (mr < B) {
@@ -228,12 +259,12 @@
             s_dhp[m * P + k] = dhp;
         }
         __syncthreads();
-        {
+        if (t_wave) {
             f32x4 acc[NTC];
             rg_mma<NTC, NCH>(s_dC, P, wx, lane, acc);
 #pragma unroll
             for (int q = 0; q < NTC; ++q) {
-                const int ct = wave + 4 * q;
+                const int ct = wave + NW * q;
                 if (ct >= ntc) continue;
                 const int n = 16 * ct + jj;
 #pragma unroll
@@ -253,12 +284,12 @@
             }
         }
         __syncthreads();
-        {
+        if (t_wave) {
             f32x4 acc[NTC];
             rg_mma<NTC, 2 * NCH>(s_dG, P2, wy, lane, acc);
 #pragma unroll
             for (int q = 0; q < NTC; ++q) {
-                const int ct = wave + 4 * q;
+                const int ct = wave + NW * q;
                 if (ct >= ntc) continue;
                 const int n = 16 * ct + jj;
 #pragma unroll
@@ -282,10 +313,19 @@
     return T >= 1 && B >= 1 && H >= 16 && H <= RG_MAXH && (H % 16) == 0 && nchain >= 1 && nchain <= 4;
 }
 
+int rowgru_waves(int requested) { return requested >= 8 ? 8 : 4; }
+
+template <int NCH, int NW>
+static void rg_launch_w(int which, const RowGruArgs& g, dim3 grid, size_t lds, hipStream_t stream) {
+    if (which == 0) hipLaunchKernelGGL((rg_fwd_kernel<NCH, NW>), grid, dim3(64 * NW), lds, stream, g);
+    else hipLaunchKernelGGL((rg_bwd_kernel<NCH, NW>), grid, dim3(64 * NW), lds, stream, g);
+}
 template <int NCH>
 static void rg_launch(int which, const RowGruArgs& g, dim3 grid, size_t lds, hipStream_t stream) {
-    if (which == 0) hipLaunchKernelGGL((rg_fwd_kernel<NCH>), grid, dim3(RG_THREADS), lds, stream, g);
-    else hipLaunchKernelGGL((rg_bwd_kernel<NCH>), grid, dim3(RG_THREADS), lds, stream, g);
+    switch (rowgru_waves(g.waves)) {
+        case 8: rg_launch_w<NCH, 8>(which, g, grid, lds, stream); break;
+        default: rg_launch_w<NCH, 4>(which, g, grid, lds, stream); break;
+    }
 }
 static int rg_dispatch(int which, const RowGruArgs& g, hipStream_t stream) {
     if (!rowgru_supported(g.T, g.B, g.H, g.nchain)) return PH_ERR_UNSUPPORTED;
diff --git a/parrot_amd/csrc/switches.h b/parrot_amd/csrc/switches.h
--- a/parrot_amd/csrc/switches.h
+++ b/parrot_amd/csrc/switches.h
@@ -10,5 +10,6 @@
 
 static inline int sw_att_dense() { return env_int("PARROT_ATT_DENSE", 0); }
 static inline int sw_pm_dataflow(int dflt) { return env_int("PARROT_PM_DATAFLOW", dflt); }
+static inline int sw_rg_waves() { return env_int("PARROT_RG_WAVES", 8); }
 static inline int sw_wk() { return env_int("PARROT_WK", 1); }
 static inline bool sw_pm_dump_plan() { return env_set("PARROT_PM_DUMP_PLAN"); }
diff --git a/parrot_amd/model.py b/parrot_amd/model.py
--- a/parrot_amd/model.py
+++ b/parrot_amd/model.py
@@ -371,6 +371,10 @@
             ctx = labels.to(torch.float32) * labels_mask[..., None]
             return ctx.contiguous()
         B, U = labels.shape
+        tables = save is not None and self._encoder_tables(B, U)
+        self._encoder_path = 'tables' if tables else 'products'
+        if tables:
+            return self._encoder_forward_tables(labels, labels_mask, save)
         P = '/encoder/encoder'
         emb = self._p('/encoder/embed_label.W')[labels.long()]
         x = emb if self.encoder_literal else emb.transpose(0, 1)
@@ -401,6 +405,8 @@
     def _encoder_backward(self, dctx, save):
         if self.encoder_type is None:
             return
+        if 'enc_lab32' in save:
+            return self._encoder_backward_tables(dctx, save)
         labels, mask, x2 = save['enc_labels'], save['enc_mask'], save['enc_x2']
         B, U = labels.shape
         P = '/encoder/encoder'
@@ -436,6 +442,89 @@
             demb = demb.transpose(0, 1)
         self._scatter_rows_add(self._g('/encoder/embed_label.W'), labels.long().reshape(-1),
                                demb.reshape(-1, demb.shape[-1]))
+
+    @property
+    def encoder_path(self):
+        return getattr(self, '_encoder_path', None)
+
+    def _encoder_tables(self, B, U):
+        return (self.encoder_type == 'bidirectional' and self.encoder_dim % 4 == 0
+                and ops.label_tables_supported(B * U, self._p('/encoder/embed_label.W').shape[0])
+                and env_int('PARROT_ENCODER_TABLES', 1) != 0)
+
+    def _enc_tables_ws(self, ws):
+        if 'P' not in ws:
+            Q, ED = self._p('/encoder/embed_label.W').shape[0], self.encoder_dim
+            f = dict(device=self._dev(), dtype=torch.float32)
+            ws['P'] = [torch.empty(Q, ED * (1 + k % 2), **f) for k in range(4)]
+            ws['S'] = [torch.empty(Q, ED * (1 + k % 2), **f) for k in range(4)]
+            ws['seg_ws'] = None
+        return ws
+
+    def _encoder_forward_tables(self, labels, labels_mask, save):
+        B, U = labels.shape
+        P = '/encoder/encoder'
+        Te, Be = self._encoder_dims(B, U)
+        ws = self._enc_tables_ws(self._enc_runner(B, U))
+        run = ws['run']
+        emb_W = self._p('/encoder/embed_label.W')
+        lab = (labels if self.encoder_literal else labels.t()).to(torch.int32).contiguous().view(-1)
+        Wg, Wc = [], []
+        with ops.gemm_precision(ops.PRECISION_F32):
+            for i, d in enumerate(('forward', 'backward')):
+                ops.gemm(emb_W, self._p(f'{P}/{d}/fork/fork_inputs.W'), bias=self._p(f'{P}/{d}/fork/fork_inputs.b'),
+                         out=ws['P'][2 * i])
+                ops.gemm(emb_W, self._p(f'{P}/{d}/fork/fork_gate_inputs.W'),
+                         bias=self._p(f'{P}/{d}/fork/fork_gate_inputs.b'), out=ws['P'][2 * i + 1])
+        ops.label_gather(lab, ws['P'], [b[i].view(Te * Be, -1) for i in range(2) for b in (run.inputs, run.gate_inputs)])
+        for i, d in enumerate(('forward', 'backward')):
+            run.h[i][0].copy_(self._p(f'{P}/{d}/gatedrecurrent.initial_state').unsqueeze(0).expand(Be, -1))
+            Wg.append(self._p(f'{P}/{d}/gatedrecurrent.state_to_gates'))
+            Wc.append(self._p(f'{P}/{d}/gatedrecurrent.state_to_state'))
+        run.bind(Wg, Wc)
+        run.forward()
+        out = torch.cat([run.h[0][1:], run.h[1][1:].flip(0)], dim=-1)
+        if not self.encoder_literal:
+            out = out.transpose(0, 1)
+        ctx = (out * labels_mask[..., None]).contiguous()
+        if save is not None:
+            save.update(enc_lab32=lab, enc_labels=labels, enc_mask=labels_mask)
+        return ctx
+
+    def _encoder_backward_tables(self, dctx, save):
+        labels, mask, lab = save['enc_labels'], save['enc_mask'], save['enc_lab32']
+        B, U = labels.shape
+        P = '/encoder/encoder'
+        ED = self.encoder_dim
+        ws = self._enc_tables_ws(self._enc_runner(B, U))
+        run = ws['run']
+        Te, Be = run.T, run.B
+        d_out = dctx * mask[..., None]
+        if not self.encoder_literal:
+            d_out = d_out.transpose(0, 1)
+        for i in range(2):
+            run.dh[i].zero_()
+        run.dh[0][1:].copy_(d_out[..., :ED])
+        run.dh[1][1:].copy_(d_out[..., ED:].flip(0))
+        run.backward()
+        ws['seg_ws'] = ops.label_segsum(lab, [b[i].view(Te * Be, -1) for i in range(2) for b in (run.dC, run.dG)],
+                                        ws['S'], ws['seg_ws'])
+        emb_W, demb = self._p('/encoder/embed_label.W'), self._g('/encoder/embed_label.W')
+        with ops.gemm_precision(ops.PRECISION_F32):
+            for i, d in enumerate(('forward', 'backward')):
+                for S, name in ((ws['S'][2 * i], 'fork_inputs'), (ws['S'][2 * i + 1], 'fork_gate_inputs')):
+                    ops.gemm(emb_W.t(), S, out=self._g(f'{P}/{d}/fork/{name}.W'), accumulate=True)
+                    ops.colsum(S, out=self._g(f'{P}/{d}/fork/{name}.b'), accumulate=True)
+                    ops.gemm(S, self._p(f'{P}/{d}/fork/{name}.W').t(), out=demb, accumulate=True)
+        for i, d in enumerate(('forward', 'backward')):
+            dC = run.dC[i].view(Te * Be, ED)
+            dG = run.dG[i].view(Te * Be, 2 * ED)
+            hprev = run.h[i][:Te] if i == 0 else run.h[i][:Te].flip(0)
+            hprev = hprev.reshape(Te * Be, ED)
+            ops.gemm(run.rh[i].view(Te * Be, ED).t(), dC,
+                     out=self._g(f'{P}/{d}/gatedrecurrent.state_to_state'), accumulate=True)
+            ops.gemm(hprev.t(), dG, out=self._g(f'{P}/{d}/gatedrecurrent.state_to_gates'), accumulate=True)
+            ops.colsum(run.dh[i][0], out=self._g(f'{P}/{d}/gatedrecurrent.initial_state'), accumulate=True)
 
     def _train_workspace(self, T, B, U):
         ws_key = ('dec', T, B, U)
diff --git a/parrot_amd/ops.py b/parrot_amd/ops.py
--- a/parrot_amd/ops.py
+++ b/parrot_amd/ops.py
@@ -350,6 +350,37 @@
     return _EmbedSumFn.apply(E, W1, idx, add)
 
 
+def _label_desc(labels32, Q, mats, field):
+    import ctypes as C
+    d = _lib.LabelTablesDesc()
+    d.N, d.Q, d.nseg = labels32.numel(), int(Q), len(mats)
+    d.labels = ptr(labels32, "labels", torch.int32)
+    for s, (m, rows) in enumerate(mats):
+        if rows.shape != (labels32.numel(), m.shape[1]) or m.shape[0] != Q:
+            raise ValueError("label tables: expected [Q, D] tables / sums and [N, D] row matrices")
+        getattr(d, field)[s], d.rows[s], d.D[s] = ptr(m, field), ptr(rows, "rows"), m.shape[1]
+    return d, C.byref(d)
+
+
+def label_tables_supported(N, Q) -> bool:
+    return bool(_lib.load().parrot_label_tables_supported(int(N), int(Q)))
+
+
+def label_gather(labels32, tables, rows):
+    d, ref = _label_desc(labels32, tables[0].shape[0], list(zip(tables, rows)), "tbl")
+    _lib.call("parrot_label_gather", ref, _stream())
+
+
+def label_segsum(labels32, rows, sums, ws=None):
+    Q = sums[0].shape[0]
+    d, ref = _label_desc(labels32, Q, list(zip(sums, rows)), "sums")
+    n_ws = int(_lib.load().parrot_label_segsum_ws_floats(d.N, Q, sum(m.shape[1] for m in sums)))
+    if ws is None or ws.numel() < n_ws:
+        ws = torch.empty(n_ws, device=labels32.device, dtype=torch.float32)
+    _lib.call("parrot_label_segsum", ref, ws.data_ptr(), ws.numel(), _stream())
+    return ws
+
+
 class _ReluMlpFn(torch.autograd.Function):
 
     @staticmethod
```

Result: faster. 901,800 frames/s (median of 6 runs) (+1.4%).
